# AIM-SE/AC-TSR

Hardware: AMD Instinct MI355X
Metric: user-sequences/sec fwd+bwd, AC-SASRec L=50 d=64, 1/2/4/8 MI355X (higher is better)
Workload: dtype f32; 1 GPU; ACSASRec full training step (spatial + adversarial calibrators, BASELINE configs[2]), synthetic 100000-item catalogue, B=512/GPU L=50 d=64 h=2 2 layers inner=256, CE loss, two-pass backward + Adam; global_batch=512, seq_len=50, hidden=64, heads=2, parallelism=dp1, launch=hipGraph replay per step, backward=two walks (reference protocol, trainer.py:672-686)

## Files before the change

### ac_tsr_amd/_lib.py

```python
from __future__ import annotations

import ctypes as C
import os
import subprocess

_HERE = os.path.dirname(os.path.abspath(__file__))
CSRC = os.path.join(_HERE, "csrc")
LIB_PATH = os.environ.get("ACATTN_LIB") or os.path.join(CSRC, "libacattn.so")
HEADER_PATH = os.path.join(os.path.dirname(_HERE), "include", "acattn.h")

ABI_VERSION = 32
MAX_MASKS = 8
NSTAT = 8
MASK_STRUCTURED, MASK_DENSE_LL, MASK_DENSE_L = 0, 1, 2
COMBINE = {"fixed": 0, "gate": 1, "annealing": 2}
RICH = {"none": 0, "fixed": 1, "trainable": 2}
RNG_EXPLICIT, RNG_COUNTER = 0, 1
FWD_AUTO, FWD_STREAM, FWD_STAGED, FWD_GENERAL = 0, 1, 2, 3
BWD_AUTO, BWD_STREAM, BWD_ROW = 0, 1, 2

_f = C.c_void_p


class Problem(C.Structure):
    _fields_ = [
        ("B", C.c_int32), ("L", C.c_int32), ("H", C.c_int32), ("n_heads", C.c_int32),
        ("q", _f), ("k", _f), ("v", _f), ("qa", _f), ("ka", _f), ("gate_logits", _f),
        ("mask_mode", C.c_int32), ("causal", C.c_int32), ("key_valid", _f), ("mask", _f),
        ("w_order", _f), ("b_order", _f), ("w_dist", _f), ("b_dist", _f), ("scalar", _f),
        ("adversarial", C.c_int32), ("combine_option", C.c_int32), ("anneal_rate", C.c_float),
        ("two_level", C.c_int32), ("rich_combine", C.c_int32), ("rich_ratio", _f),
        ("rng_mode", C.c_int32), ("p_drop", C.c_float), ("noise", _f), ("keep_after", _f), ("keep_before", _f),
        ("keep_mask", _f), ("seed", C.c_uint64), ("seed_device", _f), ("affine", _f), ("gate_is_prob", C.c_int32),
    ]


class FwdOut(C.Structure):
    _fields_ = [
        ("ctx_attacked", _f), ("ctx_calibrated", _f), ("attack_mask", _f), ("row_stats", _f),
        ("after_spatial", _f), ("before_spatial", _f), ("perturbed_attention", _f), ("calibrated_attention", _f),
        ("penalty_part", _f),
    ]


class BwdIO(C.Structure):
    _fields_ = [
        ("attack_mask", _f), ("row_stats", _f),
        ("d_ctx_attacked", _f), ("d_ctx_calibrated", _f), ("d_attack_mask", _f),
        ("dq", _f), ("dk", _f), ("dv", _f), ("dqa", _f), ("dka", _f), ("dgate_logits", _f),
        ("dw_order_part", _f), ("dw_dist_part", _f), ("dsmall_part", _f), ("part_stride", C.c_int32),
        ("active_qblocks", _f), ("attack_only", C.c_int32), ("workspace", _f), ("read_rows", _f),
        ("n_read_rows", C.c_int32), ("d_penalty_part", _f), ("dgate_summed", C.c_int32),
        ("d_ctx_calibrated2", _f), ("d_penalty_part2", _f), ("dqa2", _f), ("dka2", _f),
    ]


class SpatialBwdIO(C.Structure):
    _fields_ = [
        ("d_ctx", _f), ("dq", _f), ("dk", _f), ("dv", _f),
        ("dw_order_part", _f), ("dw_dist_part", _f), ("dsmall_part", _f), ("part_stride", C.c_int32),
        ("n_read_rows", C.c_int32), ("read_rows", _f), ("workspace", _f),
    ]


class CeProblem(C.Structure):
    _fields_ = [("B", C.c_int32), ("N", C.c_int32), ("H", C.c_int32), ("out", _f), ("table", _f), ("target", _f),
                ("coef_is_scalar", C.c_int32), ("coef_scale", C.c_float)]


class LnProblem(C.Structure):
    _fields_ = [("rows", C.c_int32), ("H", C.c_int32), ("residual_rows", C.c_int32), ("z", _f), ("residual", _f),
                ("gamma", _f), ("beta", _f), ("eps", C.c_float), ("p_drop", C.c_float), ("keep", _f),
                ("seed", C.c_uint64), ("seed_device", _f)]


LN_BWD_GRID = 512


class ProjProblem(C.Structure):
    _fields_ = [("rows", C.c_int32), ("H", C.c_int32), ("G", C.c_int32), ("x", _f), ("wq", _f), ("bq", _f), ("wk", _f),
                ("bk", _f), ("wv", _f), ("bv", _f), ("waq", _f), ("baq", _f), ("wak", _f), ("bak", _f), ("wg", _f),
                ("bg", _f), ("w_order", _f), ("b_order", _f), ("w_dist", _f), ("b_dist", _f), ("n_heads", C.c_int32),
                ("L", C.c_int32)]


class ProjOut(C.Structure):
    _fields_ = [("mq", _f), ("mk", _f), ("mv", _f), ("qa", _f), ("ka", _f), ("gate", _f), ("affine", _f),
                ("gate_prob", C.c_int32)]


class ProjBwdIO(C.Structure):
    _fields_ = [("dmq", _f), ("dmk", _f), ("dmv", _f), ("dqa", _f), ("dka", _f), ("dgate", _f), ("dmq_total", _f),
                ("dmk_total", _f), ("dx", _f), ("dx_init", _f), ("workspace", _f)]


ADAM_MAX_TENSORS = 64


class AdamGroup(C.Structure):
    _fields_ = [("n_tensors", C.c_int32), ("param", _f * ADAM_MAX_TENSORS), ("grad", _f * ADAM_MAX_TENSORS),
                ("exp_avg", _f * ADAM_MAX_TENSORS), ("exp_avg_sq", _f * ADAM_MAX_TENSORS), ("step", _f * ADAM_MAX_TENSORS),
                ("numel", C.c_int64 * ADAM_MAX_TENSORS)]


class TailProblem(C.Structure):
    _fields_ = [("rows", C.c_int32), ("H", C.c_int32), ("I", C.c_int32), ("ctx", _f), ("x", _f), ("wd", _f), ("bd", _f),
                ("g1", _f), ("b1", _f), ("w1", _f), ("bb1", _f), ("w2", _f), ("bb2", _f), ("g2", _f), ("b2", _f),
                ("eps1", C.c_float), ("eps2", C.c_float), ("p1", C.c_float), ("p2", C.c_float), ("keep1", _f),
                ("keep2", _f), ("seed1", C.c_uint64), ("seed2", C.c_uint64), ("seed_device", _f), ("src_index", _f),
                ("src_R", C.c_int32), ("src_L", C.c_int32), ("split_planes", _f)]


class TailSaved(C.Structure):
    _fields_ = [("h1", _f), ("st1", _f), ("a", _f), ("act", _f), ("h3", _f), ("st2", _f), ("out", _f),
                ("gelu_grad", _f)]


class TailBwdIO(C.Structure):
    _fields_ = [("d_out", _f), ("d_ctx", _f), ("d_x", _f), ("d_h1", _f), ("d_h2", _f), ("d_h3", _f), ("dgb_part", _f),
                ("workspace", _f)]


class EmbedProblem(C.Structure):
    _fields_ = [("rows", C.c_int32), ("L", C.c_int32), ("H", C.c_int32), ("n_table_rows", C.c_int64), ("idx", _f),
                ("table", _f), ("pos", _f), ("gamma", _f), ("beta", _f), ("eps", C.c_float), ("p_drop", C.c_float),
                ("keep", _f), ("seed", C.c_uint64), ("seed_device", _f), ("nonzero_out", _f), ("hot_id_plus1", C.c_int64)]


EMBED_BWD_CHUNKS = 8
PENALTY_WS_FLOATS = 1024
WGRAD_MAX_GROUP = 8
WGRAD_MAX_REDUCE = 32
SUMROWS_MAX_DEFER = 8

SYMBOLS = {
    "acattn_abi_version": (C.c_int, []),
    "acattn_calibrated_attention_bwd_gate_summed": (C.c_int, [C.POINTER(Problem), C.POINTER(BwdIO)]),
    "acattn_calibrated_attention_bwd_pair_supported": (C.c_int, [C.POINTER(Problem), C.POINTER(BwdIO)]),
    "acattn_last_error": (C.c_char_p, []),
    "acattn_fwd_algorithmic_bytes": (C.c_int64, [C.POINTER(Problem)]),
    "acattn_calibrated_attention_fwd": (C.c_int, [C.POINTER(Problem), C.POINTER(FwdOut), C.c_void_p]),
    "acattn_calibrated_attention_bwd": (C.c_int, [C.POINTER(Problem), C.POINTER(BwdIO), C.c_void_p]),
    "acattn_spatial_attention_bwd": (C.c_int, [C.POINTER(Problem), C.POINTER(SpatialBwdIO), C.c_void_p]),
    "acattn_spatial_attention_bwd_workspace_bytes": (C.c_int64, [C.POINTER(Problem)]),
    "acattn_spatial_affines": (C.c_int, [C.POINTER(Problem), _f, C.c_void_p]),
    "acattn_full_sort_ce_workspace_bytes": (C.c_int64, [C.POINTER(CeProblem)]),
    "acattn_full_sort_ce_fwd": (C.c_int, [C.POINTER(CeProblem), _f, _f, _f, C.c_void_p]),
    "acattn_full_sort_ce_fwd_dir": (C.c_int, [C.POINTER(CeProblem), _f, _f, _f, _f, C.c_void_p]),
    "acattn_full_sort_ce_bwd": (C.c_int, [C.POINTER(CeProblem), _f, _f, _f, _f, _f, C.c_void_p]),
    "acattn_full_sort_ce_products": (C.c_int, [C.c_int]),
    "acattn_linear_products": (C.c_int, [C.c_int]),
    "acattn_dropout_add_layernorm_fwd": (C.c_int, [C.POINTER(LnProblem), _f, _f, C.c_void_p]),
    "acattn_dropout_add_layernorm_bwd": (C.c_int, [C.POINTER(LnProblem), _f, _f, _f, _f, _f, C.c_void_p]),
    "acattn_embed_layernorm_fwd": (C.c_int, [C.POINTER(EmbedProblem), _f, _f, C.c_void_p]),
    "acattn_embed_layernorm_bwd": (C.c_int, [C.POINTER(EmbedProblem), _f, _f, C.c_int64, _f, _f, _f, C.c_void_p]),
    "acattn_projections_supported": (C.c_int, [C.c_int32, C.c_int32]),
    "acattn_projections_bwd_workspace_bytes": (C.c_int64, [C.POINTER(ProjProblem)]),
    "acattn_projections_fwd": (C.c_int, [C.POINTER(ProjProblem), C.POINTER(ProjOut), C.c_void_p]),
    "acattn_projections_qkv_supported": (C.c_int, [C.c_int32]),
    "acattn_projections_qkv_fwd": (C.c_int, [C.POINTER(ProjProblem), C.POINTER(ProjOut), C.c_void_p]),
    "acattn_projections_bwd": (C.c_int, [C.POINTER(ProjProblem), C.POINTER(ProjBwdIO), C.c_void_p]),
    "acattn_layer_tail_supported": (C.c_int, [C.c_int32, C.c_int32]),
    "acattn_layer_tail_fwd": (C.c_int, [C.POINTER(TailProblem), C.POINTER(TailSaved), C.c_void_p]),
    "acattn_layer_tail_bwd": (C.c_int, [C.POINTER(TailProblem), C.POINTER(TailSaved), C.POINTER(TailBwdIO), C.c_void_p]),
    "acattn_layer_tail_bwd_partial_rows": (C.c_int32, [C.c_int32]),
    "acattn_layer_tail_bwd_partial_rows_for": (C.c_int32, [C.c_int32, C.c_int32]),
    "acattn_layer_tail_bwd_workspace_bytes": (C.c_int64, [C.c_int32, C.c_int32]),
    "acattn_select_layer_tail_blocks": (C.c_int, [C.c_int]),
    "acattn_layer_tail_split_bytes": (C.c_int64, [C.c_int32, C.c_int32, C.c_int32]),
    "acattn_layer_tail_split_weights": (C.c_int, [C.POINTER(TailProblem), C.c_void_p, C.c_void_p]),
    "acattn_adam_step": (C.c_int, [C.POINTER(AdamGroup), C.c_double, C.c_double, C.c_double, C.c_double, C.c_double, _f,
                                   C.c_void_p]),
    "acattn_dense_ce_fwd": (C.c_int, [_f, C.c_int64, C.c_int64, _f, _f, _f, C.c_void_p]),
    "acattn_dense_ce_bwd": (C.c_int, [_f, _f, _f, _f, C.c_int64, C.c_int64, _f, C.c_void_p]),
    "acattn_step_inputs": (C.c_int, [C.POINTER(C.c_void_p), C.POINTER(C.c_void_p), C.POINTER(C.c_int64), C.c_int32, C.c_void_p,
                                     C.c_void_p, C.c_void_p, C.c_int32, C.c_void_p]),
    "acattn_sum_rows": (C.c_int, [_f, _f, C.c_int32, C.c_int32, C.c_int32, C.c_void_p]),
    "acattn_sum_rows_pair": (C.c_int, [_f, _f, C.c_int32, C.c_int32, C.c_int32, _f, _f, C.c_int32, C.c_int32, C.c_int32, C.c_void_p]),
    "acattn_mask_penalty_fwd": (C.c_int, [_f, C.c_int64, _f, _f, C.c_void_p]),
    "acattn_mask_penalty_partial": (C.c_int, [_f, C.c_int64, _f, C.c_void_p]),
    "acattn_mask_penalty_partial_multi": (C.c_int, [C.c_void_p, C.c_int32, C.c_int64, _f, C.c_void_p]),
    "acattn_mask_penalty_bwd_scaled_multi": (C.c_int, [C.c_void_p, _f, _f, C.c_float, C.c_int64, C.c_void_p, C.c_int32,
                                                       C.c_void_p]),
    "acattn_attacked_loss_finish": (C.c_int, [_f, C.c_int32, _f, C.c_int32, C.c_int64, C.c_float, _f, _f, C.c_int32,
                                              C.c_void_p]),
    "acattn_mask_penalty_rows": (C.c_int, [_f, C.c_int32, C.c_int32, C.c_int32, _f, C.c_void_p]),
    "acattn_attacked_loss_finish_rows": (C.c_int, [_f, C.c_int32, C.c_void_p, C.c_int32, C.c_int32, C.c_float, _f, _f, C.c_int32,
                                                  C.c_void_p]),
    "acattn_mask_penalty_drows": (C.c_int, [_f, _f, C.c_float, C.c_int32, C.c_void_p, C.c_int32, C.c_void_p]),
    "acattn_mask_penalty_drows_dir": (C.c_int, [_f, _f, C.c_float, C.c_int32, C.c_void_p, C.c_int32, _f, _f, C.c_int32, C.c_void_p]),
    "acattn_mask_penalty_bwd_scaled": (C.c_int, [_f, _f, _f, C.c_float, C.c_int64, _f, C.c_void_p]),
    "acattn_mask_penalty_bwd": (C.c_int, [_f, _f, _f, C.c_int64, _f, C.c_void_p]),
    "acattn_linear_wgrad_workspace_bytes": (C.c_int64, [C.c_int64, C.c_int32, C.c_int32]),
    "acattn_linear_wgrad_grouped": (C.c_int, [C.c_void_p, C.c_void_p, C.c_void_p, C.c_void_p, C.c_void_p, C.c_void_p,
                                               C.c_int32, C.c_int64, _f, C.c_void_p]),
    "acattn_linear_wgrad": (C.c_int, [_f, _f, C.c_int64, C.c_int32, C.c_int32, _f, _f, _f, C.c_void_p]),
    "acattn_linear_wgrad_grouped_partial": (C.c_int, [C.c_void_p, C.c_void_p, C.c_void_p, C.c_void_p, C.c_void_p, C.c_int32,
                                                       C.c_int64, C.c_void_p, C.c_void_p, C.c_void_p, C.c_void_p, C.c_void_p]),
    "acattn_linear_wgrad_reduce_many": (C.c_int, [C.c_void_p, C.c_void_p, C.c_void_p, C.c_void_p, C.c_void_p, C.c_void_p,
                                                   C.c_void_p, C.c_int32, C.c_void_p, C.c_void_p, C.c_void_p, C.c_void_p,
                                                   C.c_int32, C.c_void_p]),
    "acattn_select_forward_kernel": (C.c_int, [C.c_int]),
    "acattn_select_backward_kernel": (C.c_int, [C.c_int]),
    "acattn_calibrated_attention_bwd_workspace_bytes": (C.c_int64, [C.POINTER(Problem)]),
    "acattn_rng_materialize": (C.c_int, [C.c_int32, C.c_int32, C.c_int32, C.c_uint64, C.c_float, _f, _f, _f, _f,
                                         C.c_void_p]),
}

_lib = None


class AcattnError(RuntimeError):
    pass


def build(verbose: bool = False) -> str:
    jobs = str(min(8, os.cpu_count() or 1))
    res = subprocess.run(["make", "-C", CSRC, "-j", jobs], capture_output=not verbose, text=True)
    if res.returncode != 0:
        raise AcattnError("building libacattn.so failed:\n" + (res.stdout or "") + (res.stderr or ""))
    return LIB_PATH


def load() -> C.CDLL:
    global _lib
    if _lib is not None:
        return _lib
    if not os.path.exists(LIB_PATH):
        raise AcattnError(
            f"{LIB_PATH} is missing: the HIP extension has not been built. Run "
            "`make -C ac_tsr_amd/csrc` (or __graft_entry__.build()). There is no CPU / eager fallback.")
    lib = C.CDLL(LIB_PATH)
    for name, (res, args) in SYMBOLS.items():
        fn = getattr(lib, name)
        fn.restype = res
        fn.argtypes = args
    got = lib.acattn_abi_version()
    if got != ABI_VERSION:
        raise AcattnError(f"libacattn.so ABI {got} != binding ABI {ABI_VERSION}; rebuild")
    _lib = lib
    return lib


def check(rc: int, what: str) -> None:
    if rc == 0:
        return
    msg = load().acattn_last_error().decode()
    if rc < 0 and "not a multiple of the number of attention" in msg:
        raise ValueError(msg)
    if rc < 0 and ("unknown combine_option" in msg or "unknown rich_calibrated_combine" in msg):
        raise KeyError(msg)
    raise AcattnError(f"{what} failed (rc={rc}): {msg}")
```

### ac_tsr_amd/csrc/acattn_api.hip

```cpp
#include <stdint.h>
#include <stdio.h>
#include <string.h>

#include <algorithm>

#include "acattn_common.h"

namespace {
thread_local char g_err[256] = "";

int fail(const char* msg) {
  snprintf(g_err, sizeof(g_err), "%s", msg);
  return -1;
}

int check_problem(const acattn_problem* p) {
  if (!p) return fail("problem is NULL");
  if (p->B < 1 || p->L < 1 || p->H < 1 || p->n_heads < 1) return fail("B, L, H, n_heads must be positive");
  if (p->H % p->n_heads != 0)
    return fail("The hidden size is not a multiple of the number of attention heads");
  const int dh = p->H / p->n_heads;
  if (dh != 16 && dh != 32 && dh != 64 && dh != 128) return fail("unsupported head size: dh must be 16, 32, 64 or 128");
  if (p->L > 208) return fail("unsupported sequence length: L must be <= 208");
  if (!p->q || !p->k || !p->v) return fail("q, k, v must be non-NULL");
// ... 133 lines not shown
                                   (hipStream_t)stream);
  if (rc > 0) snprintf(g_err, sizeof(g_err), "HIP launch failed: %s", hipGetErrorString((hipError_t)rc));
  return rc;
}

static int check_ce(const acattn_ce_problem* p) {
  if (!p) return fail("ce problem is NULL");
  if (p->B < 1 || p->N < 1) return fail("B and N must be positive");
  if (p->H != 64 && p->H != 128 && p->H != 256) return fail("unsupported hidden size for the fused cross-entropy: H must be 64, 128 or 256");
  if (!p->out || !p->table || !p->target) return fail("out, table, target must be non-NULL");
  return 0;
}

int64_t acattn_full_sort_ce_workspace_bytes(const acattn_ce_problem* p) {
  if (!p || (p->H != 64 && p->H != 128 && p->H != 256)) return -1;
  return acattn_ce_ws_bytes(*p);
}

int acattn_full_sort_ce_fwd(const acattn_ce_problem* p, void* workspace, float* lse, float* row_loss, void* stream) {
  if (int rc = check_ce(p)) return rc;
  if (!workspace || !lse || !row_loss) return fail("workspace, lse, row_loss must be non-NULL");
  const int rc = acattn_launch_ce_fwd(*p, workspace, lse, row_loss, (hipStream_t)stream);
  if (rc > 0) snprintf(g_err, sizeof(g_err), "HIP launch failed: %s", hipGetErrorString((hipError_t)rc));
  return rc;
}

int acattn_full_sort_ce_fwd_dir(const acattn_ce_problem* p, void* workspace, float* lse, float* row_loss, float* dir,
                                void* stream) {
  if (int rc = check_ce(p)) return rc;
  if (!workspace || !lse || !row_loss || !dir) return fail("workspace, lse, row_loss, dir must be non-NULL");
  const int rc = acattn_launch_ce_fwd_dir(*p, workspace, lse, row_loss, dir, (hipStream_t)stream);
  if (rc > 0) snprintf(g_err, sizeof(g_err), "HIP launch failed: %s", hipGetErrorString((hipError_t)rc));
  return rc;
}

int acattn_full_sort_ce_bwd(const acattn_ce_problem* p, const float* lse, const float* coef, void* workspace,
                            float* d_out, float* d_table, void* stream) {
  if (int rc = check_ce(p)) return rc;
  if (!workspace || !lse || !coef || !d_out) return fail("workspace, lse, coef, d_out must be non-NULL");
  const int rc = acattn_launch_ce_bwd(*p, lse, coef, workspace, d_out, d_table, (hipStream_t)stream);
  if (rc > 0) snprintf(g_err, sizeof(g_err), "HIP launch failed: %s", hipGetErrorString((hipError_t)rc));
  return rc;
}

int acattn_full_sort_ce_products(int mode) { return acattn_ce_products_choice(mode); }

int acattn_linear_products(int mode) { return acattn_linear_products_choice(mode); }

static int check_ln(const acattn_ln_problem* p) {
  if (!p) return fail("ln problem is NULL");
  if (p->rows < 1) return fail("rows must be positive");
  if (p->H != 64 && p->H != 128 && p->H != 256) return fail("unsupported hidden size for the fused LayerNorm: H must be 64, 128 or 256");
  if (p->residual_rows < 1 || p->rows % p->residual_rows != 0) return fail("residual_rows must divide rows");
  if (!p->z || !p->residual || !p->gamma || !p->beta) return fail("z, residual, gamma, beta must be non-NULL");
  if (p->p_drop < 0.f || p->p_drop >= 1.f) return fail("p_drop must lie in [0, 1)");
  return 0;
}

int acattn_dropout_add_layernorm_fwd(const acattn_ln_problem* p, float* y, float* stats, void* stream) {
  if (int rc = check_ln(p)) return rc;
  if (!y || !stats) return fail("y and stats must be non-NULL");
  const int rc = acattn_launch_ln_fwd(*p, y, stats, (hipStream_t)stream);
  if (rc > 0) snprintf(g_err, sizeof(g_err), "HIP launch failed: %s", hipGetErrorString((hipError_t)rc));
  return rc;
}

int acattn_dropout_add_layernorm_bwd(const acattn_ln_problem* p, const float* dy, const float* stats, float* dz,
                                     float* dres, float* dgb_part, void* stream) {
  if (int rc = check_ln(p)) return rc;
  if (!dy || !stats) return fail("dy and stats must be non-NULL");
  const int rc = acattn_launch_ln_bwd(*p, dy, stats, dz, dres, dgb_part, (hipStream_t)stream);
  if (rc > 0) snprintf(g_err, sizeof(g_err), "HIP launch failed: %s", hipGetErrorString((hipError_t)rc));
  return rc;
}

static int check_proj(const acattn_proj_problem* p) {
  if (!p) return fail("problem must be non-NULL");
  if (p->rows < 1) return fail("rows must be positive");
  if (!acattn_proj_supported(p->H, p->G)) return fail("projections: hidden_size must be 64, 128 or 256 and the gate at most 256 wide");
  if (!p->x || !p->wq || !p->bq || !p->wk || !p->bk || !p->wv || !p->bv || !p->waq || !p->baq || !p->wak || !p->bak)
    return fail("projections: input and parameters must be non-NULL");
  if ((p->wg != nullptr) != (p->bg != nullptr) || (p->wg != nullptr) != (p->G > 0))
    return fail("projections: gate weight, bias and width go together");
  return 0;
}

int acattn_projections_supported(int32_t H, int32_t G) { return acattn_proj_supported(H, G) ? 1 : 0; }

int64_t acattn_projections_bwd_workspace_bytes(const acattn_proj_problem* p) {
  if (!p || !acattn_proj_supported(p->H, p->G)) return -1;
  return acattn_proj_bwd_ws_bytes(*p);
}

int acattn_projections_fwd(const acattn_proj_problem* p, const acattn_proj_out* out, void* stream) {
  if (int rc = check_proj(p)) return rc;
  if (!out || !out->mq || !out->mk || !out->mv || !out->qa || !out->ka) return fail("projections: outputs must be non-NULL");
  if ((p->wg != nullptr) != (out->gate != nullptr)) return fail("projections: gate output goes with the gate parameters");
  if (out->affine) {
    if (!p->w_order || !p->b_order || !p->w_dist || !p->b_dist) return fail("projections: affine planes need the spatial calibrator's parameters");
    if (p->n_heads < 1 || p->H % p->n_heads != 0 || (p->H / p->n_heads) % 16 != 0) return fail("projections: affine planes need a head size that is a multiple of 16");
    if (p->L < 1 || p->rows % p->L != 0) return fail("projections: affine planes need rows = B * L");
  }
  const int rc = acattn_launch_proj_fwd(*p, *out, (hipStream_t)stream);
  if (rc > 0) snprintf(g_err, sizeof(g_err), "HIP launch failed: %s", hipGetErrorString((hipError_t)rc));
  return rc;
}

int acattn_projections_qkv_supported(int32_t H) { return acattn_proj_qkv_supported(H) ? 1 : 0; }

int acattn_projections_qkv_fwd(const acattn_proj_problem* p, const acattn_proj_out* out, void* stream) {
  if (!p) return fail("problem must be non-NULL");
  if (p->rows < 1) return fail("rows must be positive");
  if (!acattn_proj_qkv_supported(p->H)) return fail("projections (q, k, v only): hidden_size must be 64 with the split products on");
  if (!p->x || !p->wq || !p->bq || !p->wk || !p->bk || !p->wv || !p->bv) return fail("projections: input and parameters must be non-NULL");
  if (!out || !out->mq || !out->mk || !out->mv) return fail("projections: outputs must be non-NULL");
  if (out->qa || out->ka || out->gate) return fail("projections (q, k, v only): qa, ka and gate outputs must be NULL");
  if (out->affine) {
    if (!p->w_order || !p->b_order || !p->w_dist || !p->b_dist) return fail("projections: affine planes need the spatial calibrator's parameters");
    if (p->n_heads < 1 || p->H % p->n_heads != 0 || (p->H / p->n_heads) % 16 != 0) return fail("projections: affine planes need a head size that is a multiple of 16");
    if (p->L < 1 || p->rows % p->L != 0) return fail("projections: affine planes need rows = B * L");
  }
  const int rc = acattn_launch_proj_qkv_fwd(*p, *out, (hipStream_t)stream);
  if (rc > 0) snprintf(g_err, sizeof(g_err), "HIP launch failed: %s", hipGetErrorString((hipError_t)rc));
  return rc;
}

int acattn_projections_bwd(const acattn_proj_problem* p, const acattn_proj_bwd_io* io, void* stream) {
  if (int rc = check_proj(p)) return rc;
  if (!io) return fail("io must be non-NULL");
  if (!io->dmq_total && !io->dmk_total && !io->dx) return fail("projections backward: nothing to compute");
  const int rc = acattn_launch_proj_bwd(*p, *io, (hipStream_t)stream);
  if (rc > 0) snprintf(g_err, sizeof(g_err), "HIP launch failed: %s", hipGetErrorString((hipError_t)rc));
  return rc;
}

static int check_tail(const acattn_tail_problem* p, const acattn_tail_saved* s) {
  if (!p || !s) return fail("problem and saved must be non-NULL");
  if (p->rows < 1) return fail("rows must be positive");
  if (!acattn_tail_supported(p->H, p->I)) return fail("layer tail: (hidden_size, inner_size) must be (64, 256), (64, 128), (128, 512), (128, 256) or (256, 1024)");
  if (!p->ctx || !p->x || !p->wd || !p->bd || !p->g1 || !p->b1 || !p->w1 || !p->bb1 || !p->w2 || !p->bb2 || !p->g2 || !p->b2)
    return fail("layer tail: inputs and parameters must be non-NULL");
  if (!(p->p1 >= 0.f && p->p1 < 1.f) || !(p->p2 >= 0.f && p->p2 < 1.f)) return fail("dropout probabilities must be in [0, 1)");
  if (!s->h1 || !s->st1 || !s->a || !s->h3 || !s->st2) return fail("layer tail: saved tensors must be non-NULL");
  if (p->src_index && (p->src_R < 1 || p->src_L < 1)) return fail("layer tail: src_index needs src_R, src_L >= 1");
  if (p->split_planes && p->H != 64) return fail("layer tail: split_planes is for hidden 64 only");
  if (((uintptr_t)p->split_planes & 15) != 0) return fail("layer tail: split_planes must be 16-byte aligned");
  return 0;
}

int acattn_layer_tail_supported(int32_t H, int32_t I) { return acattn_tail_supported(H, I) ? 1 : 0; }

int32_t acattn_layer_tail_bwd_partial_rows(int32_t rows) { return acattn_tail_bwd_partial_rows(rows); }
int32_t acattn_layer_tail_bwd_partial_rows_for(int32_t rows, int32_t H) { return acattn_tail_bwd_partial_rows_h(rows, H); }
int64_t acattn_layer_tail_bwd_workspace_bytes(int32_t H, int32_t I) {
  return acattn_tail_supported(H, I) ? acattn_tail_bwd_ws_bytes(H, I) : -1;
}

int64_t acattn_layer_tail_split_bytes(int32_t H, int32_t I, int32_t rows) {
  return acattn_tail_supported(H, I) && rows > 0 ? acattn_tail_split_bytes(H, I, rows) : 0;
}

int acattn_layer_tail_split_weights(const acattn_tail_problem* p, void* planes, void* stream) {
  if (!p || !planes || !p->wd || !p->w1 || !p->w2) return fail("layer tail split planes: problem, weights and planes must be non-NULL");
  if (p->H != 64 || (p->I != 256 && p->I != 128)) return fail("layer tail split planes: hidden 64, inner 256 or 128 only");
  if (((uintptr_t)planes & 15) != 0) return fail("layer tail split planes: planes must be 16-byte aligned");
  const int rc = acattn_launch_tail_split(*p, planes, (hipStream_t)stream);
  if (rc > 0) snprintf(g_err, sizeof(g_err), "HIP launch failed: %s", hipGetErrorString((hipError_t)rc));
  return rc;
}

int acattn_select_layer_tail_blocks(int nb) {
  if (nb < 0 || nb > 2) return fail("rows per wave: 0 (automatic), 1 or 2 blocks of 16");
  return acattn_select_tail_nb(nb);
}

int acattn_layer_tail_fwd(const acattn_tail_problem* p, const acattn_tail_saved* saved, void* stream) {
  if (int rc = check_tail(p, saved)) return rc;
  if (!saved->act || !saved->out) return fail("layer tail forward: act and out must be non-NULL");
  const int rc = acattn_launch_tail_fwd(*p, *saved, (hipStream_t)stream);
  if (rc > 0) snprintf(g_err, sizeof(g_err), "HIP launch failed: %s", hipGetErrorString((hipError_t)rc));
  return rc;
}

int acattn_layer_tail_bwd(const acattn_tail_problem* p, const acattn_tail_saved* saved, const acattn_tail_bwd_io* io,
                          void* stream) {
  if (int rc = check_tail(p, saved)) return rc;
  if (!io || !io->d_out) return fail("layer tail backward: d_out must be non-NULL");
  const int rc = acattn_launch_tail_bwd(*p, *saved, *io, (hipStream_t)stream);
  if (rc > 0) snprintf(g_err, sizeof(g_err), "HIP launch failed: %s", hipGetErrorString((hipError_t)rc));
  return rc;
}

int acattn_dense_ce_fwd(const float* logits, int64_t rows, int64_t N, const int64_t* target, float* lse, float* row_loss,
                        void* stream) {
  if (!logits || !target || !lse || !row_loss) return fail("dense CE: logits, target, lse, row_loss must be non-NULL");
  if (rows < 1 || N < 1) return fail("dense CE: rows and N must be positive");
  const int rc = acattn_launch_dense_ce_fwd(logits, rows, N, target, lse, row_loss, (hipStream_t)stream);
  if (rc > 0) snprintf(g_err, sizeof(g_err), "HIP launch failed: %s", hipGetErrorString((hipError_t)rc));
  return rc;
}
int acattn_dense_ce_bwd(const float* logits, const float* lse, const int64_t* target, const float* coef, int64_t rows, int64_t N,
                        float* d_logits, void* stream) {
  if (!logits || !lse || !target || !coef || !d_logits) return fail("dense CE backward: every pointer must be non-NULL");
  if (rows < 1 || N < 1) return fail("dense CE: rows and N must be positive");
  const int rc = acattn_launch_dense_ce_bwd(logits, lse, target, coef, rows, N, d_logits, (hipStream_t)stream);
  if (rc > 0) snprintf(g_err, sizeof(g_err), "HIP launch failed: %s", hipGetErrorString((hipError_t)rc));
  return rc;
}

int acattn_step_inputs(const void* const* src, void* const* dst, const int64_t* bytes, int32_t n_copies, int64_t* counter,
                       const int64_t* item_length, int64_t* last_row, int32_t n_rows, void* stream) {
  if (n_copies < 0 || n_copies > ACATTN_MAX_COPIES) return fail("step inputs: 0 .. ACATTN_MAX_COPIES copies");
  if (n_copies > 0 && (!src || !dst || !bytes)) return fail("step inputs: src, dst, bytes must be non-NULL");
  for (int k = 0; k < n_copies; ++k)
    if (bytes[k] > 0 && (!src[k] || !dst[k])) return fail("step inputs: NULL copy operand");
  if ((item_length == nullptr) != (last_row == nullptr)) return fail("step inputs: item_length and last_row come together");
  if (last_row && n_rows < 1) return fail("step inputs: n_rows must be positive");
  const int rc = acattn_launch_step_inputs(src, dst, bytes, n_copies, counter, item_length, last_row, n_rows, (hipStream_t)stream);
  if (rc > 0) snprintf(g_err, sizeof(g_err), "HIP launch failed: %s", hipGetErrorString((hipError_t)rc));
  return rc;
}

int acattn_sum_rows(const float* x, float* out, int32_t batch, int32_t R, int32_t C, void* stream) {
  if (!x || !out) return fail("x and out must be non-NULL");
  if (batch < 1 || R < 1 || C < 1) return fail("batch, R, C must be positive");
  const int rc = acattn_launch_sum_rows(x, out, batch, R, C, (hipStream_t)stream);
  if (rc > 0) snprintf(g_err, sizeof(g_err), "HIP launch failed: %s", hipGetErrorString((hipError_t)rc));
  return rc;
}

int acattn_sum_rows_pair(const float* x1, float* out1, int32_t batch1, int32_t R1, int32_t C1, const float* x2, float* out2,
                         int32_t batch2, int32_t R2, int32_t C2, void* stream) {
  if (!x1 || !out1 || !x2 || !out2) return fail("x and out must be non-NULL");
  if (batch1 < 1 || R1 < 1 || C1 < 1 || batch2 < 1 || R2 < 1 || C2 < 1) return fail("batch, R, C must be positive");
  const int rc = acattn_launch_sum_rows_pair(x1, out1, batch1, R1, C1, x2, out2, batch2, R2, C2, (hipStream_t)stream);
  if (rc > 0) snprintf(g_err, sizeof(g_err), "HIP launch failed: %s", hipGetErrorString((hipError_t)rc));
  return rc;
}

static int check_embed(const acattn_embed_problem* p) {
  if (!p) return fail("embed problem is NULL");
  if (p->rows < 1 || p->L < 1 || p->rows % p->L != 0) return fail("rows must be a positive multiple of L");
  if (p->H != 64 && p->H != 128 && p->H != 256) return fail("unsupported hidden size for the fused embedding front end: H must be 64, 128 or 256");
  if (p->n_table_rows < 1) return fail("n_table_rows must be positive");
  if (!p->idx || !p->table || !p->gamma || !p->beta) return fail("idx, table, gamma, beta must be non-NULL");
  if (p->p_drop < 0.f || p->p_drop >= 1.f) return fail("p_drop must lie in [0, 1)");
  return 0;
}

// ... 229 lines not shown
```

### ac_tsr_amd/csrc/acattn_common.h

```cpp
#pragma once
#include <hip/hip_runtime.h>
#include <stdint.h>

#include <type_traits>

#include "acattn.h"

typedef float f4 __attribute__((ext_vector_type(4)));
typedef float f4u __attribute__((ext_vector_type(4), aligned(4)));

#define ACATTN_NEG_INF (-__builtin_inff())
#define ACATTN_MASK_FILL (-10000.0f)
#define ACATTN_LOG_EPS (1e-24f)

__device__ __forceinline__ float quad_sum(float x) {
  auto r = __builtin_amdgcn_permlane16_swap(__float_as_uint(x), __float_as_uint(x), false, false);
  x = __uint_as_float(r[0]) + __uint_as_float(r[1]);
  auto s = __builtin_amdgcn_permlane32_swap(__float_as_uint(x), __float_as_uint(x), false, false);
  return __uint_as_float(s[0]) + __uint_as_float(s[1]);
}

__device__ __forceinline__ float quad_max(float x) {
  auto r = __builtin_amdgcn_permlane16_swap(__float_as_uint(x), __float_as_uint(x), false, false);
  x = fmaxf(__uint_as_float(r[0]), __uint_as_float(r[1]));
// ... 177 lines not shown
  x ^= x >> 16;
  x += key.b;
  return (rng_word(x, 0xB5297A4Du, 0x85EBCA77u) >> 12) & 0xFu;
}

__device__ __forceinline__ f4 keep_scale4(uint32_t bits, float keep_scale) {
  f4 s;
#pragma unroll
  for (int r = 0; r < 4; ++r) s[r] = ((bits >> r) & 1u) ? keep_scale : 0.f;
  return s;
}
__device__ __forceinline__ int sbit(uint32_t bits, int idx) {
  int m = __builtin_amdgcn_sbfe(bits, idx, 1);
  asm("" : "+v"(m));
  return m;
}
__device__ __forceinline__ float keep_and(float x, uint32_t bits, int r) {
  return __uint_as_float(__float_as_uint(x) & (uint32_t)sbit(bits, r));
}

__device__ __forceinline__ void store_out4(float* p, const f4 v) { __builtin_nontemporal_store(v, (f4*)p); }
__device__ __forceinline__ void store_out1(float* p, const float v) { __builtin_nontemporal_store(v, p); }

__device__ __forceinline__ bool qblock_has_ctx(const acattn_bwd_io& IO, int b, int qb) {
  if (IO.active_qblocks) return (IO.active_qblocks[b] >> qb) & 1u;
  if (IO.read_rows) {
    for (int r = 0; r < IO.n_read_rows; ++r)
      if ((int)(IO.read_rows[(size_t)b * IO.n_read_rows + r] >> 4) == qb) return true;
    return false;
  }
  return true;
}

__device__ __forceinline__ bool qblock_active(const acattn_bwd_io& IO, int b, int qb) {
  if (IO.d_attack_mask || IO.d_penalty_part) return true;
  if (IO.active_qblocks) return (IO.active_qblocks[b] >> qb) & 1u;
  if (IO.read_rows) {
    for (int r = 0; r < IO.n_read_rows; ++r)
      if ((int)(IO.read_rows[(size_t)b * IO.n_read_rows + r] >> 4) == qb) return true;
    return false;
  }
  return true;
}

__device__ __forceinline__ void decode_block(int bid, int B, int nh, int& b, int& h) {
  if ((B & 7) == 0) {
    const int grp = bid / (8 * nh), rem = bid - grp * 8 * nh;
    h = rem >> 3;
    b = grp * 8 + (rem & 7);
  } else {
    b = bid / nh;
    h = bid - b * nh;
  }
}

int acattn_launch_fwd(const acattn_problem& p, const acattn_fwd_out& o, hipStream_t stream);
int acattn_fwd_kernel_choice(int which);
int acattn_bwd_kernel_choice(int which);
int64_t acattn_bwd_stream_ws_bytes(const acattn_problem& p);
int acattn_launch_bwd(const acattn_problem& p, const acattn_bwd_io& io, hipStream_t stream);
bool acattn_bwd_gate_summed(const acattn_problem& p, const acattn_bwd_io& io);
bool acattn_bwd_pair_supported(const acattn_problem& p, const acattn_bwd_io& io);
int64_t acattn_spatial_bwd_ws_bytes(const acattn_problem& p);
int acattn_launch_spatial_bwd(const acattn_problem& p, const acattn_spatial_bwd_io& io, hipStream_t stream);
int acattn_launch_spatial_affines(const acattn_problem& p, float* affine, hipStream_t stream);
int acattn_launch_rng(int B, int nh, int L, uint64_t seed, float p_drop, float* noise, uint8_t* keep_after,
                      uint8_t* keep_mask, uint8_t* keep_before, hipStream_t stream);
int64_t acattn_ce_ws_bytes(const acattn_ce_problem& p);
int acattn_launch_ce_fwd(const acattn_ce_problem& p, void* ws, float* lse, float* row_loss, hipStream_t stream);
int acattn_launch_ce_fwd_dir(const acattn_ce_problem& p, void* ws, float* lse, float* row_loss, float* dir,
                             hipStream_t stream);
int acattn_launch_ce_bwd(const acattn_ce_problem& p, const float* lse, const float* coef, void* ws, float* d_out,
                         float* d_table, hipStream_t stream);
int acattn_launch_ln_fwd(const acattn_ln_problem& p, float* y, float* stats, hipStream_t stream);
int acattn_launch_ln_bwd(const acattn_ln_problem& p, const float* dy, const float* stats, float* dz, float* dres,
                         float* dgb_part, hipStream_t stream);
int acattn_launch_sum_rows(const float* x, float* out, int batch, int R, int C, hipStream_t stream);
int acattn_launch_sum_rows_pair(const float* x1, float* out1, int batch1, int R1, int C1, const float* x2, float* out2,
                                int batch2, int R2, int C2, hipStream_t stream);
void acattn_set_error(const char* msg);
bool acattn_proj_supported(int H, int G);
int64_t acattn_proj_bwd_ws_bytes(const acattn_proj_problem& p);
int acattn_launch_proj_fwd(const acattn_proj_problem& p, const acattn_proj_out& o, hipStream_t stream);
bool acattn_proj_qkv_supported(int H);
int acattn_launch_proj_qkv_fwd(const acattn_proj_problem& p, const acattn_proj_out& o, hipStream_t stream);
int acattn_launch_proj_bwd(const acattn_proj_problem& p, const acattn_proj_bwd_io& io, hipStream_t stream);
bool acattn_tail_supported(int H, int I);
int acattn_tail_bwd_partial_rows(int rows);
int acattn_tail_bwd_partial_rows_h(int rows, int H);
int64_t acattn_tail_bwd_ws_bytes(int H, int I);
int acattn_select_tail_nb(int nb);
int64_t acattn_tail_split_bytes(int H, int I, int rows);
int acattn_launch_tail_split(const acattn_tail_problem& p, void* planes, hipStream_t stream);
int acattn_launch_tail_fwd(const acattn_tail_problem& p, const acattn_tail_saved& s, hipStream_t stream);
int acattn_launch_tail_bwd(const acattn_tail_problem& p, const acattn_tail_saved& s, const acattn_tail_bwd_io& io,
                           hipStream_t stream);
int64_t acattn_linear_wgrad_ws_bytes(int64_t M, int K, int N);
int acattn_launch_linear_wgrad(const float* const* x, const float* const* dy, const int* K, const int* N,
                               float* const* dw, float* const* db, int n_items, int64_t M, void* ws, hipStream_t stream,
                               int* P_out = nullptr, long long* w_off_out = nullptr, long long* b_off_out = nullptr);
int acattn_launch_linear_wgrad_reduce_many(const float* const* part_w, const float* const* part_b, const int* K, const int* N,
                                           const int* P, float* const* dw, float* const* db, int n_items,
                                           const float* const* sr_x, float* const* sr_out, const int* sr_R, const int* sr_C,
                                           int n_sr, hipStream_t stream);
int acattn_launch_embed_fwd(const acattn_embed_problem& p, float* y, float* stats, hipStream_t stream);
int acattn_launch_embed_bwd(const acattn_embed_problem& p, const float* dy, const float* stats, int64_t padding_idx,
                            float* d_table, float* d_pos_part, float* dgb_part, hipStream_t stream);
int acattn_launch_penalty_fwd(const float* m, int64_t n, float* ws, float* norm, hipStream_t stream);
int acattn_launch_penalty_partial(const float* m, int64_t n, float* part, hipStream_t stream);
void acattn_penalty_written_set(bool v);
bool acattn_penalty_written();
int acattn_launch_penalty_rows(const float* m, int B, int nh, int L, float* pen, hipStream_t stream);
int acattn_launch_attacked_loss_finish_rows(const float* row_loss, int B, const float* const* pen, int n_masks, int count,
                                            float weight, float* out, float* scale_buf, int n_scale, hipStream_t stream);
int acattn_launch_penalty_drows(const float* norms, const float* d_loss, float scale, int count, float* const* d_pen,
                                int n_masks, hipStream_t stream, const float* dir = nullptr, float* d_out = nullptr, int n_dir = 0);
int acattn_launch_attacked_loss_finish(const float* row_loss, int B, const float* part, int n_masks, int64_t mask_numel,
                                       float weight, float* out, float* scale_buf, int n_scale, hipStream_t stream);
int acattn_launch_penalty_bwd_scaled(const float* m, const float* norm, const float* d_loss, float scale, int64_t n,
                                     float* d_m, hipStream_t stream);
int acattn_launch_penalty_bwd(const float* m, const float* norm, const float* d_norm, int64_t n, float* d_m,
                              hipStream_t stream);
int acattn_launch_zero(float* p, size_t n, hipStream_t stream);
int64_t acattn_ce6_rows_bytes(const acattn_ce_problem& p);
int acattn_launch_ce6_sweep(const acattn_ce_problem& p, const float* lse, const float* coef, float* slab, float* d_table,
                            float2* part, void* rows_ws, int n_wg, int n_left, bool dir, hipStream_t stream);
int acattn_launch_ce6_onehot_reduce(const acattn_ce_problem& p, const float* coef, const float* slab, int n_slabs, float* d_out,
                                    float* d_table, hipStream_t stream);
int acattn_launch_ce6_fwd_sweep(const acattn_ce_problem& p, float2* part, void* rows_ws, int n_wg, int n_left, hipStream_t stream);
int acattn_ce_products_choice(int mode);
int acattn_linear_products_choice(int mode);
int acattn_launch_dense_ce_fwd(const float* logits, int64_t rows, int64_t N, const int64_t* target, float* lse, float* row_loss,
                               hipStream_t stream);
int acattn_launch_dense_ce_bwd(const float* logits, const float* lse, const int64_t* target, const float* coef, int64_t rows,
                               int64_t N, float* d_logits, hipStream_t stream);
int acattn_launch_step_inputs(const void* const* src, void* const* dst, const int64_t* bytes, int n, int64_t* counter,
                              const int64_t* item_length, int64_t* last_row, int n_rows, hipStream_t stream);
int acattn_launch_penalty_partial_multi(const float* const* m, int n_masks, int64_t n, float* part, hipStream_t stream);
int acattn_launch_penalty_bwd_scaled_multi(const float* const* m, const float* norms, const float* d_loss, float scale,
                                           int64_t n, float* const* d_m, int n_masks, hipStream_t stream);
int acattn_launch_adam_step(const acattn_adam_group& g, double lr, double beta1, double beta2, double eps,
                            double weight_decay, int* done, hipStream_t stream);
```

### ac_tsr_amd/csrc/acattn_proj.hip

```cpp
#include <stdlib.h>
#include <string.h>

#include <algorithm>
#include <type_traits>

#include "acattn_common.h"
#include "acattn_split.h"
#include "acattn_wstage.h"

namespace {

template <int NB>
struct Rows {
  int row[NB];
  bool ok[NB];
};

template <int NB>
__device__ __forceinline__ Rows<NB> wave_rows(int R) {
  Rows<NB> w;
  const int c = threadIdx.x & 15;
#pragma unroll
  for (int nb = 0; nb < NB; ++nb) {
    const int r = (blockIdx.x * NB + nb) * 16 + c;
// ... 751 lines not shown
  f4 in[NB][DT], tot[NB][DT];
  auto zero = [&](f4 (&v)[NB][DT]) {
#pragma unroll
    for (int nb = 0; nb < NB; ++nb)
#pragma unroll
      for (int t = 0; t < DT; ++t) v[nb][t] = f4{0.f, 0.f, 0.f, 0.f};
  };
  auto masked_store_rows = [&](float* out, const f4 (&v)[NB][DT]) {
#pragma unroll
    for (int nb = 0; nb < NB; ++nb)
      if (W.ok[nb])
#pragma unroll
        for (int t = 0; t < DT; ++t) *(f4*)(out + (size_t)W.row[nb] * H + 16 * t + 4 * g) = v[nb][t];
  };
  if (h_dmq) load_rows<DT, NB>(IO.dmq, W, g, tot); else zero(tot);
  if (h_dqa) load_rows<DT, NB>(IO.dqa, W, g, in);
  st.commit();
  if (h_dqa) staged_keep<DT, NB, false>(st, waqT, nullptr, in, tot, after_qa);
  if (h_gate) {
    static_assert(DT == KT || DT == 2 * KT, "");
    for (int kt = 0; kt < GT; ++kt) {
      f4 d[NB];
#pragma unroll
      for (int nb = 0; nb < NB; ++nb) {
        const int j0 = 16 * kt + 4 * g;
        const float* src = IO.dgate + (size_t)W.row[nb] * P.G + j0;
        f4 v = {0.f, 0.f, 0.f, 0.f};
        if (j0 + 3 < P.G) {
          v = *(const f4u*)src;
        } else {
#pragma unroll
          for (int r = 0; r < 4; ++r)
            if (j0 + r < P.G) v[r] = src[r];
        }
        d[nb] = v;
      }
#pragma unroll
      for (int half = 0; half < DT / KT; ++half) {
        f4 frag[KT], b;
        st.fetch(frag, b);
        if (half + 1 < DT / KT)
          st.request_cols(wgT + (size_t)(16 * KT) * ldg * (half + 1), ldg, kt);
        else if (kt + 1 < GT)
          st.request_cols(wgT, ldg, kt + 1);
        else
          after_q_total();
        PIN_ORDER();
#pragma unroll
        for (int r = 0; r < 4; ++r)
#pragma unroll
          for (int nt = 0; nt < KT; ++nt)
#pragma unroll
            for (int nb = 0; nb < NB; ++nb) {
              if (half == 0) tot[nb][nt] = mfma16(frag[nt][r], d[nb][r], tot[nb][nt]);
              else tot[nb][DT - KT + nt] = mfma16(frag[nt][r], d[nb][r], tot[nb][DT - KT + nt]);
            }
        PIN_ORDER();
        st.commit();
      }
    }
  }
  if (h_qt) masked_store_rows(IO.dmq_total, tot);
  if (h_dmk) load_rows<DT, NB>(IO.dmk, W, g, tot); else zero(tot);
  if (h_dka) {
    load_rows<DT, NB>(IO.dka, W, g, in);
    staged_keep<DT, NB, false>(st, wakT, nullptr, in, tot, after_k_total);
  }
  if (h_kt) masked_store_rows(IO.dmk_total, tot);
  if (h_dx) {
    f4 (&dx)[NB][DT] = in;
    if (IO.dx_init) load_rows<DT, NB>(IO.dx_init, W, g, dx); else zero(dx);
    staged_keep<DT, NB, false>(st, wkT, nullptr, tot, dx, [&] { first(wqT); });
    load_rows<DT, NB>(IO.dmq_total, W, g, tot);
    staged_keep<DT, NB, false>(st, wqT, nullptr, tot, dx, [&] { if (h_dmv) first(wvT); else st.has_bias = false; });
    if (h_dmv) {
      load_rows<DT, NB>(IO.dmv, W, g, tot);
      staged_keep<DT, NB, false>(st, wvT, nullptr, tot, dx, [&] { st.has_bias = false; });
    }
    masked_store_rows(IO.dx, dx);
  }
}

constexpr int SPW = 4;
constexpr int SPLIT_MAT = 4 * 2 * 3 * 64;
constexpr int SPLIT_LDS = 6 * SPLIT_MAT * (int)sizeof(b8);

__device__ __forceinline__ int kperm(int s, int g, int j) { return 32 * s + 16 * (j >> 2) + 4 * g + (j & 3); }

template <bool T>
__device__ __forceinline__ void split_raw(const float* w, int n_out, int nt, int c, int g, float (&v)[2][8]) {
#pragma unroll
  for (int s = 0; s < 2; ++s) {
    if constexpr (!T) {
      const float* row = w + (size_t)min(16 * nt + c, n_out - 1) * 64 + 32 * s + 4 * g;
      const f4 lo = *(const f4*)row, hi = *(const f4*)(row + 16);
#pragma unroll
      for (int r = 0; r < 4; ++r) {
        v[s][r] = lo[r];
        v[s][4 + r] = hi[r];
      }
    } else {
#pragma unroll
      for (int j = 0; j < 8; ++j) {
        const int k = kperm(s, g, j);
        const float t = w[(size_t)min(k, n_out - 1) * 64 + 16 * nt + c];
        v[s][j] = k < n_out ? t : 0.f;
      }
    }
  }
}

__device__ __forceinline__ void split_store(const float (&v)[2][8], b8* mat, int nt, int lane) {
#pragma unroll
  for (int s = 0; s < 2; ++s) {
    b8 p[3];
    split8(v[s], p[0], p[1], p[2]);
#pragma unroll
    for (int q = 0; q < 3; ++q) mat[((nt * 2 + s) * 3 + q) * 64 + lane] = p[q];
  }
}

template <int NB>
__device__ __forceinline__ void split_rows(const f4 (&v)[NB][4], b8 (&b)[NB][2][3]) {
#pragma unroll
  for (int nb = 0; nb < NB; ++nb)
#pragma unroll
    for (int s = 0; s < 2; ++s) {
      float x[8];
#pragma unroll
      for (int r = 0; r < 4; ++r) {
        x[r] = v[nb][2 * s][r];
        x[4 + r] = v[nb][2 * s + 1][r];
      }
      split8(x, b[nb][s][0], b[nb][s][1], b[nb][s][2]);
    }
}

template <int NB, int NT = 4>
__device__ __forceinline__ void split_product(const b8* mat, int lane, const b8 (&b)[NB][2][3], f4 (&acc)[NB][4]) {
#pragma unroll
  for (int nt = 0; nt < NT; ++nt) {
    b8 a[2][3];
#pragma unroll
    for (int s = 0; s < 2; ++s)
#pragma unroll
      for (int q = 0; q < 3; ++q) a[s][q] = mat[((nt * 2 + s) * 3 + q) * 64 + lane];
#pragma unroll
    for (int s = 0; s < 2; ++s)
#pragma unroll
      for (int nb = 0; nb < NB; ++nb) acc[nb][nt] = mfma_split(a[s], b[nb][s], acc[nb][nt]);
  }
}

template <int NB>
__device__ __forceinline__ Rows<NB> split_rows_of(int R, int wave) {
  Rows<NB> w;
  const int c = threadIdx.x & 15;
#pragma unroll
  for (int nb = 0; nb < NB; ++nb) {
    const int r = ((blockIdx.x * SPW + wave) * NB + nb) * 16 + c;
    w.ok[nb] = r < R;
    w.row[nb] = r < R ? r : R - 1;
  }
  return w;
}

template <int NB>
__global__ void __launch_bounds__(64 * SPW) proj_split_fwd_kernel(const acattn_proj_problem P, const acattn_proj_out O) {
// ... 107 lines not shown
  split_product<NB>(wsp + 2 * SPLIT_MAT, lane, xs, acc);
  store_rows<4, NB>(O.mv, W, g, acc);
}

template <int NB, int MODE>
__global__ void __launch_bounds__(64 * SPW) proj_split_bwd_kernel(const acattn_proj_problem P, const acattn_proj_bwd_io IO) {
  extern __shared__ b8 wsp[];
  const bool h_dmq = MODE == 1 || (MODE == 0 && IO.dmq), h_dmk = MODE == 1 || (MODE == 0 && IO.dmk);
  const bool h_dmv = MODE == 1 || (MODE == 0 && IO.dmv);
  const bool h_dqa = MODE != 0 || IO.dqa, h_dka = MODE != 0 || IO.dka, h_dx = MODE != 0 || IO.dx;
  const bool h_qt = MODE != 0 || IO.dmq_total, h_kt = MODE != 0 || IO.dmk_total;
  const bool gate = MODE != 2 && IO.dgate && P.wg;
  const int lane = threadIdx.x & 63, wave = threadIdx.x >> 6, c = lane & 15, g = lane >> 4;
  const Rows<NB> W = split_rows_of<NB>(P.rows, wave);
  {
    const float* src[6] = {P.waq, gate ? P.wg : P.waq, P.wq, P.wak, P.wk, P.wv};
    const bool need[6] = {h_dqa, gate, h_dx, h_dka, h_dx, h_dx && h_dmv};
    float v[6][2][8];
#pragma unroll
    for (int m = 0; m < 6; ++m)
      if (need[m]) split_raw<true>(src[m], m == 1 ? P.G : 64, wave, c, g, v[m]);
#pragma unroll
    for (int m = 0; m < 6; ++m)
      if (need[m]) split_store(v[m], wsp + m * SPLIT_MAT, wave, lane);
  }
  auto zero = [&](f4 (&v)[NB][4]) {
#pragma unroll
    for (int nb = 0; nb < NB; ++nb)
#pragma unroll
      for (int t = 0; t < 4; ++t) v[nb][t] = f4{0.f, 0.f, 0.f, 0.f};
  };
  f4 in[NB][4], dq[NB][4], dk[NB][4], dx[NB][4];
  b8 bs[NB][2][3];
  if (IO.dx_init && h_dx) load_rows<4, NB>(IO.dx_init, W, g, dx); else zero(dx);
  if (h_dmq) load_rows<4, NB>(IO.dmq, W, g, dq); else zero(dq);
  if (h_dqa) load_rows<4, NB>(IO.dqa, W, g, in);
  __syncthreads();

  if (h_dqa) {
    split_rows<NB>(in, bs);
    split_product<NB>(wsp, lane, bs, dq);
  }
  if (gate) {
#pragma unroll
    for (int nb = 0; nb < NB; ++nb)
#pragma unroll
      for (int s = 0; s < 2; ++s) {
        float x[8];
#pragma unroll
        for (int j = 0; j < 8; ++j) {
          const int k = kperm(s, g, j);
          const float t = IO.dgate[(size_t)W.row[nb] * P.G + min(k, P.G - 1)];
          x[j] = k < P.G ? t : 0.f;
        }
        split8(x, bs[nb][s][0], bs[nb][s][1], bs[nb][s][2]);
      }
    split_product<NB>(wsp + SPLIT_MAT, lane, bs, dq);
  }
  if (h_qt) store_rows<4, NB>(IO.dmq_total, W, g, dq);
  if (h_dx) {
    split_rows<NB>(dq, bs);
    split_product<NB>(wsp + 2 * SPLIT_MAT, lane, bs, dx);
  }

  if (h_dmk) load_rows<4, NB>(IO.dmk, W, g, dk); else zero(dk);
  if (h_dka) {
    load_rows<4, NB>(IO.dka, W, g, in);
    split_rows<NB>(in, bs);
    split_product<NB>(wsp + 3 * SPLIT_MAT, lane, bs, dk);
  }
  if (h_kt) store_rows<4, NB>(IO.dmk_total, W, g, dk);
  if (h_dx) {
    split_rows<NB>(dk, bs);
    split_product<NB>(wsp + 4 * SPLIT_MAT, lane, bs, dx);
    if (h_dmv) {
      load_rows<4, NB>(IO.dmv, W, g, in);
      split_rows<NB>(in, bs);
      split_product<NB>(wsp + 5 * SPLIT_MAT, lane, bs, dx);
    }
    store_rows<4, NB>(IO.dx, W, g, dx);
  }
}

int rows_per_wave(int rows) {
  static const int forced = getenv("ACATTN_PROJ_ROWS_PER_WAVE") ? atoi(getenv("ACATTN_PROJ_ROWS_PER_WAVE")) : 0;
  if (forced == 16 || forced == 32) return forced;
  return rows >= 16384 ? 32 : 16;
}

}

bool acattn_proj_supported(int H, int G) { return (H == 64 || H == 128 || H == 256) && G >= 0 && G <= 256; }

int64_t acattn_proj_bwd_ws_bytes(const acattn_proj_problem& p) {
  if (p.H == 64) return 0;
  return ((int64_t)5 * p.H * p.H + (int64_t)p.H * ((p.G + 15) & ~15)) * (int64_t)sizeof(float);
}

namespace {
template <int H>
int launch_wide_fwd(const acattn_proj_problem& p, const acattn_proj_out& o, hipStream_t stream) {
#ifdef ACATTN_PROJ_NB1
  constexpr int NB = 1;
#else
  constexpr int NB = H == 128 ? 2 : 1;
#endif
  static const bool per_wave = getenv("ACATTN_PROJ_PER_WAVE") != nullptr;
  if (!per_wave) {
    const int blocks = (p.rows + 16 * NB * NWV - 1) / (16 * NB * NWV);
    hipLaunchKernelGGL((proj_staged_fwd_kernel<H, NB>), dim3(blocks), dim3(64 * NWV), 0, stream, p, o);
    return (int)hipGetLastError();
  }
  const int blocks = (p.rows + 16 * NB - 1) / (16 * NB);
  hipLaunchKernelGGL((proj_wide_fwd_kernel<H, NB>), dim3(blocks), dim3(64), 0, stream, p, o);
  return (int)hipGetLastError();
}
template <int H>
int launch_wide_bwd(const acattn_proj_problem& p, const acattn_proj_bwd_io& io, hipStream_t stream) {
  constexpr int NB = H == 128 ? 2 : 1;
  if (!io.workspace) {
    acattn_set_error("projections backward at hidden 128 / 256 needs acattn_proj_bwd_io.workspace");
    return -1;
  }
  if (io.dx && !io.dmq_total) {
    acattn_set_error("projections backward at hidden 128 / 256: dx needs dmq_total (it is read back as a source of dx)");
    return -1;
  }
  float* wt = (float*)io.workspace;
  TransposeJob J;
  const float* src[6] = {p.wq, p.wk, p.wv, p.waq, p.wak, p.wg};
  for (int k = 0; k < 6; ++k) {
    J.src[k] = src[k];
    J.n_out[k] = k < 5 ? p.H : p.G;
  }
  const int max_out = std::max(p.H, (p.G + 15) & ~15);
  hipLaunchKernelGGL(transpose_weights_kernel, dim3(max_out / 16, p.H / 16, p.wg ? 6 : 5), dim3(256), 0, stream, J, p.H, wt);
  const bool outs = io.dx && io.dmq_total && io.dmk_total, attack = io.dqa && io.dka;
  const bool all_in = attack && io.dmq && io.dmk && io.dmv && (io.dgate || !p.wg);
  const bool attack_only = attack && !io.dmq && !io.dmk && !io.dmv && !io.dgate;
  const int mode = !outs ? 0 : all_in ? 1 : attack_only ? 2 : 0;
  static const bool per_wave = getenv("ACATTN_PROJ_PER_WAVE") != nullptr;
  if (!per_wave) {
    const int wgs = (p.rows + 16 * NB * NWV - 1) / (16 * NB * NWV);
    if (mode == 1)
      hipLaunchKernelGGL((proj_staged_bwd_kernel<H, NB, 1>), dim3(wgs), dim3(64 * NWV), 0, stream, p, io, (const float*)wt);
    else if (mode == 2)
      hipLaunchKernelGGL((proj_staged_bwd_kernel<H, NB, 2>), dim3(wgs), dim3(64 * NWV), 0, stream, p, io, (const float*)wt);
    else
      hipLaunchKernelGGL((proj_staged_bwd_kernel<H, NB, 0>), dim3(wgs), dim3(64 * NWV), 0, stream, p, io, (const float*)wt);
    return (int)hipGetLastError();
  }
  const int blocks = (p.rows + 16 * NB - 1) / (16 * NB);
  if (mode == 1)
    hipLaunchKernelGGL((proj_wide_bwd_kernel<H, NB, 1>), dim3(blocks), dim3(64), 0, stream, p, io, (const float*)wt);
  else if (mode == 2)
    hipLaunchKernelGGL((proj_wide_bwd_kernel<H, NB, 2>), dim3(blocks), dim3(64), 0, stream, p, io, (const float*)wt);
  else
    hipLaunchKernelGGL((proj_wide_bwd_kernel<H, NB, 0>), dim3(blocks), dim3(64), 0, stream, p, io, (const float*)wt);
  return (int)hipGetLastError();
}
}

namespace {
int g_linear_products = -1;
int linear_products() {
  if (g_linear_products < 0) {
    const char* e = getenv("ACATTN_LINEAR_PRODUCTS");
    g_linear_products = e && !strcmp(e, "fp32") ? 0 : 1;
  }
  return g_linear_products;
}
bool use_split(const acattn_proj_problem& p) { return p.H == 64 && (!p.wg || p.G <= 64) && linear_products() == 1; }

template <class K>
bool allow_split_lds(K kern) {
  return hipFuncSetAttribute((const void*)kern, hipFuncAttributeMaxDynamicSharedMemorySize, SPLIT_LDS) == hipSuccess;
}

template <int NB>
int launch_split_fwd(const acattn_proj_problem& p, const acattn_proj_out& o, hipStream_t stream) {
  static const bool lds_ok = allow_split_lds(proj_split_fwd_kernel<NB>);
  if (!lds_ok) return (int)hipErrorInvalidValue;
  const int wgs = (p.rows + 16 * NB * SPW - 1) / (16 * NB * SPW);
  hipLaunchKernelGGL((proj_split_fwd_kernel<NB>), dim3(wgs), dim3(64 * SPW), SPLIT_LDS, stream, p, o);
  return (int)hipGetLastError();
}

template <int NB, int MODE>
int launch_split_bwd(const acattn_proj_problem& p, const acattn_proj_bwd_io& io, hipStream_t stream) {
  static const bool lds_ok = allow_split_lds(proj_split_bwd_kernel<NB, MODE>);
  if (!lds_ok) return (int)hipErrorInvalidValue;
  const int wgs = (p.rows + 16 * NB * SPW - 1) / (16 * NB * SPW);
  hipLaunchKernelGGL((proj_split_bwd_kernel<NB, MODE>), dim3(wgs), dim3(64 * SPW), SPLIT_LDS, stream, p, io);
  return (int)hipGetLastError();
}
}

int acattn_linear_products_choice(int mode) {
  const int old = linear_products();
  if (mode >= 0 && mode <= 1) g_linear_products = mode;
  return old;
}

int acattn_launch_proj_fwd(const acattn_proj_problem& p, const acattn_proj_out& o, hipStream_t stream) {
  if (p.H == 128) return launch_wide_fwd<128>(p, o, stream);
  if (p.H == 256) return launch_wide_fwd<256>(p, o, stream);
  const int rpw = rows_per_wave(p.rows), blocks = (p.rows + rpw - 1) / rpw;
  if (use_split(p)) return rpw == 32 ? launch_split_fwd<2>(p, o, stream) : launch_split_fwd<1>(p, o, stream);
  if (rpw == 32)
    hipLaunchKernelGGL((proj_fwd_kernel<64, 2>), dim3(blocks), dim3(64), 0, stream, p, o);
  else
    hipLaunchKernelGGL((proj_fwd_kernel<64, 1>), dim3(blocks), dim3(64), 0, stream, p, o);
  return (int)hipGetLastError();
}

bool acattn_proj_qkv_supported(int H) { return H == 64 && linear_products() == 1; }

namespace {
template <int NB>
int launch_split_qkv_fwd(const acattn_proj_problem& p, const acattn_proj_out& o, hipStream_t stream) {
  static const bool lds_ok = hipFuncSetAttribute((const void*)proj_split_qkv_fwd_kernel<NB>,
                                                 hipFuncAttributeMaxDynamicSharedMemorySize, SPLIT_QKV_LDS) == hipSuccess;
  if (!lds_ok) return (int)hipErrorInvalidValue;
  const int wgs = (p.rows + 16 * NB * SPW - 1) / (16 * NB * SPW);
  hipLaunchKernelGGL((proj_split_qkv_fwd_kernel<NB>), dim3(wgs), dim3(64 * SPW), SPLIT_QKV_LDS, stream, p, o);
  return (int)hipGetLastError();
}
}

int acattn_launch_proj_qkv_fwd(const acattn_proj_problem& p, const acattn_proj_out& o, hipStream_t stream) {
  if (!acattn_proj_qkv_supported(p.H)) {
    acattn_set_error("projections (q, k, v only): hidden_size must be 64 with the split products on");
    return -1;
  }
  return rows_per_wave(p.rows) == 32 ? launch_split_qkv_fwd<2>(p, o, stream) : launch_split_qkv_fwd<1>(p, o, stream);
}

int acattn_launch_proj_bwd(const acattn_proj_problem& p, const acattn_proj_bwd_io& io, hipStream_t stream) {
  if (p.H == 128) return launch_wide_bwd<128>(p, io, stream);
  if (p.H == 256) return launch_wide_bwd<256>(p, io, stream);
  const int rpw = rows_per_wave(p.rows), blocks = (p.rows + rpw - 1) / rpw;
  const bool outs = io.dx && io.dmq_total && io.dmk_total, attack = io.dqa && io.dka;
  const bool all_in = attack && io.dmq && io.dmk && io.dmv && (io.dgate || !p.wg);
  const bool attack_only = attack && !io.dmq && !io.dmk && !io.dmv && !io.dgate;
  const int mode = !outs ? 0 : all_in ? 1 : attack_only ? 2 : 0;
  if (use_split(p)) {
    if (rpw == 32) {
      if (mode == 1) return launch_split_bwd<2, 1>(p, io, stream);
      if (mode == 2) return launch_split_bwd<2, 2>(p, io, stream);
      return launch_split_bwd<2, 0>(p, io, stream);
    }
    if (mode == 1) return launch_split_bwd<1, 1>(p, io, stream);
    if (mode == 2) return launch_split_bwd<1, 2>(p, io, stream);
    return launch_split_bwd<1, 0>(p, io, stream);
  }
#define LAUNCH(NB, MODE) hipLaunchKernelGGL((proj_bwd_kernel<64, NB, MODE>), dim3(blocks), dim3(64), 0, stream, p, io)
  if (rpw == 32) {
    if (mode == 1) LAUNCH(2, 1); else if (mode == 2) LAUNCH(2, 2); else LAUNCH(2, 0);
  } else {
    if (mode == 1) LAUNCH(1, 1); else if (mode == 2) LAUNCH(1, 2); else LAUNCH(1, 0);
  }
#undef LAUNCH
  return (int)hipGetLastError();
}
```

### ac_tsr_amd/csrc/acattn_split.h

```cpp
#pragma once

#include "acattn_common.h"

namespace {

typedef __bf16 b8 __attribute__((ext_vector_type(8)));

#define ACATTN_SPLIT_TERMS(X) X(0, 2) X(1, 1) X(2, 0) X(0, 1) X(1, 0) X(0, 0)

__device__ __forceinline__ f4 mfma_bf(const b8 a, const b8 b, const f4 c) {
  return __builtin_amdgcn_mfma_f32_16x16x32_bf16(a, b, c, 0, 0, 0);
}

__device__ __forceinline__ void split8(const float (&x)[8], b8& p0, b8& p1, b8& p2) {
#pragma unroll
  for (int j = 0; j < 8; ++j) {
    const __bf16 a = (__bf16)x[j];
    const float r1 = x[j] - (float)a;
    const __bf16 b = (__bf16)r1;
    const float r2 = r1 - (float)b;
    p0[j] = a;
    p1[j] = b;
    p2[j] = (__bf16)r2;
  }
}

__device__ __forceinline__ f4 mfma_split(const b8 (&a)[3], const b8 (&b)[3], f4 acc) {
#define ACATTN_SPLIT_TERM(p, q) acc = mfma_bf(a[p], b[q], acc);
  ACATTN_SPLIT_TERMS(ACATTN_SPLIT_TERM)
#undef ACATTN_SPLIT_TERM
  return acc;
}

}
```

### ac_tsr_amd/csrc/acattn_tail.hip

```cpp
#include <stdlib.h>
#include <string.h>

#include <algorithm>

#include "acattn_common.h"
#include "acattn_rowops.h"
#include "acattn_split.h"
#include "acattn_wstage.h"

int acattn_tail_bwd_partial_rows(int rows);
int acattn_tail_bwd_partial_rows_h(int rows, int H);

namespace {

int g_tail_nb = getenv("ACATTN_TAIL_BLOCKS") ? atoi(getenv("ACATTN_TAIL_BLOCKS")) : 0;
bool split_slabs(int rows) {
  static const int limit = getenv("ACATTN_TAIL_SPLIT_ROWS") ? atoi(getenv("ACATTN_TAIL_SPLIT_ROWS")) : 4096;
  return g_tail_nb == 0 && rows <= limit;
}
#ifndef ACATTN_TAIL64_WAVES
#define ACATTN_TAIL64_WAVES 3
#endif
bool staged64(int rows) {
  static const bool per_wave = getenv("ACATTN_TAIL_PER_WAVE") != nullptr;
// ... 412 lines not shown
        const size_t o = (size_t)W.row[nb] * H + 16 * t + 4 * g;
        z[t] = *(const f4*)(S.h1 + o);
        res[t] = *(const f4*)(P.x + (size_t)W.src[nb] * H + 16 * t + 4 * g);
        keep[t] = row_keep_scale(P.p1, P.keep1, P.seed1 + step, W.row[nb], 4 * t + g, H);
      }
      const float2 st = *(const float2*)(S.st1 + 2 * (size_t)W.row[nb]);
      ln_backward<DT>(z, res, keep, P.g1, st.x, st.y, da[nb], W.ok[nb], g, dz, acc_g, acc_b);
#pragma unroll
      for (int t = 0; t < DT; ++t) {
        const size_t o = (size_t)W.row[nb] * H + 16 * t + 4 * g;
        dh1[nb][t] = dz[t] * keep[t];
        if (W.ok[nb]) {
          if (IO.d_x) store_grad(IO.d_x + (size_t)W.src[nb] * H + 16 * t + 4 * g, dz[t], P.src_index != nullptr);
          if (IO.d_h1) *(f4*)(IO.d_h1 + o) = dh1[nb][t];
        }
      }
    }
    if (part) {
      store_partial<DT>(part, acc_g, c, g);
      store_partial<DT>(part + H, acc_b, c, g);
    }
  }
  if (IO.d_ctx) {
    f4 dc[NB][DT];
#pragma unroll
    for (int nb = 0; nb < NB; ++nb)
#pragma unroll
      for (int nt = 0; nt < DT; ++nt) dc[nb][nt] = f4{0.f, 0.f, 0.f, 0.f};
    f4 wdt[DT][DT];
#pragma unroll
    for (int nt = 0; nt < DT; ++nt)
#pragma unroll
      for (int t = 0; t < DT; ++t)
#pragma unroll
        for (int r = 0; r < 4; ++r) wdt[nt][t][r] = P.wd[(size_t)(16 * t + 4 * g + r) * H + 16 * nt + c];
#pragma unroll
    for (int t = 0; t < DT; ++t)
#pragma unroll
      for (int r = 0; r < 4; ++r)
#pragma unroll
        for (int nt = 0; nt < DT; ++nt)
#pragma unroll
          for (int nb = 0; nb < NB; ++nb) dc[nb][nt] = mfma16(wdt[nt][t][r], dh1[nb][t][r], dc[nb][nt]);
#pragma unroll
    for (int nb = 0; nb < NB; ++nb)
      if (W.ok[nb])
#pragma unroll
        for (int nt = 0; nt < DT; ++nt) store_grad(IO.d_ctx + (size_t)W.src[nb] * H + 16 * nt + 4 * g, dc[nb][nt], P.src_index != nullptr);
  }
}


template <int I>
struct TailPlanes {
  static constexpr int SQ = 64 * 64 * 3 / 8, RECT = I * 64 * 3 / 8;
  static constexpr int FWD_D = 0, FWD_1 = SQ, FWD_2 = SQ + RECT;
  static constexpr int BWD_D = SQ + 2 * RECT, BWD_1 = 2 * SQ + 2 * RECT, BWD_2 = 2 * SQ + 3 * RECT;
  static constexpr int TOTAL = 2 * SQ + 4 * RECT;
};

__device__ __forceinline__ int tail_kperm(int s, int g, int j) { return 32 * s + 16 * (j >> 2) + 4 * g + (j & 3); }

template <int I>
__global__ void __launch_bounds__(256) tail_split_planes_kernel(const float* wd, const float* w1, const float* w2, b8* planes) {
  using L = TailPlanes<I>;
  const int mtx = blockIdx.y, which = mtx % 3;
  const bool T = mtx >= 3;
  const float* w = which == 0 ? wd : which == 1 ? w1 : w2;
  const int M = which == 0 ? 64 : ((which == 1) != T ? I : 64), K = (which == 0 ? 64 * 64 : 64 * I) / M, KS = K / 32;
  b8* dst = planes + (mtx == 0 ? L::FWD_D : mtx == 1 ? L::FWD_1 : mtx == 2 ? L::FWD_2 : mtx == 3 ? L::BWD_D : mtx == 4 ? L::BWD_1 : L::BWD_2);
  const int idx = blockIdx.x * 256 + threadIdx.x;
  if (idx >= (M / 16) * KS * 64) return;
  const int lane = idx & 63, f = idx >> 6, mt = f / KS, s = f % KS, c = lane & 15, g = lane >> 4, m = 16 * mt + c;
  float x[8];
#pragma unroll
  for (int j = 0; j < 8; ++j) {
    const int k = tail_kperm(s, g, j);
    x[j] = T ? w[(size_t)k * M + m] : w[(size_t)m * K + k];
  }
  b8 p[3];
  split8(x, p[0], p[1], p[2]);
#pragma unroll
  for (int q = 0; q < 3; ++q) dst[((size_t)f * 3 + q) * 64 + lane] = p[q];
}

template <int KS>
__device__ __forceinline__ void load_frag(const b8* mat, int mt, int s, int lane, b8 (&a)[3]) {
#pragma unroll
  for (int q = 0; q < 3; ++q) a[q] = mat[((mt * KS + s) * 3 + q) * 64 + lane];
}

__device__ __forceinline__ void split_tiles(const f4 lo, const f4 hi, b8 (&b)[3]) {
  float x[8];
#pragma unroll
  for (int r = 0; r < 4; ++r) {
    x[r] = lo[r];
    x[4 + r] = hi[r];
  }
  split8(x, b[0], b[1], b[2]);
}

template <int NB>
__device__ __forceinline__ void split_rows64(const f4 (&v)[NB][4], b8 (&b)[NB][2][3]) {
#pragma unroll
  for (int nb = 0; nb < NB; ++nb)
#pragma unroll
    for (int s = 0; s < 2; ++s) split_tiles(v[nb][2 * s], v[nb][2 * s + 1], b[nb][s]);
}

template <int NB>
__device__ __forceinline__ void split_square(const b8* mat, int lane, const b8 (&b)[NB][2][3], f4 (&acc)[NB][4]) {
#pragma unroll
  for (int nt = 0; nt < 4; ++nt)
#pragma unroll
    for (int s = 0; s < 2; ++s) {
      b8 w[3];
      load_frag<2>(mat, nt, s, lane, w);
#pragma unroll
      for (int nb = 0; nb < NB; ++nb) acc[nb][nt] = mfma_split(w, b[nb][s], acc[nb][nt]);
    }
}

template <int H, int I, int NB, int NW = 1>
__global__ void __launch_bounds__(64 * NW) tail_split_fwd_kernel(const acattn_tail_problem P, const acattn_tail_saved S) {
  static_assert(H == 64 && (NW == 1 || NB == 1), "hidden 64; the slab split works on one row block");
  using L = TailPlanes<I>;
  constexpr int DT = 4, NP = I / 32, NJ = NP / NW;
  static_assert(NP % NW == 0 && NJ >= 1, "whole pairs per wave");
  const int lane = threadIdx.x & 63, c = lane & 15, g = lane >> 4;
  const int wave = NW > 1 ? __builtin_amdgcn_readfirstlane(threadIdx.x >> 6) : 0;
  const Rows<NB> W = wave_rows<NB>(P);
  const uint64_t step = P.seed_device ? *P.seed_device : 0ull;
  const b8* planes = (const b8*)P.split_planes;
  const b8 *pw1 = planes + L::FWD_1, *pw2 = planes + L::FWD_2;

  struct W1Pair {
    b8 w[2][2][3];
    f4 b[2];
  };
  auto load_w1 = [&](int p, W1Pair& d) {
#pragma unroll
    for (int tt = 0; tt < 2; ++tt) {
#pragma unroll
      for (int s = 0; s < 2; ++s) load_frag<2>(pw1, 2 * p + tt, s, lane, d.w[tt][s]);
      d.b[tt] = *(const f4*)(P.bb1 + 32 * p + 16 * tt + 4 * g);
    }
  };
  W1Pair w1b[2];
  load_w1(wave, w1b[0]);

  f4 h1[NB][DT], a[NB][DT];
  {
    f4 cb[NB][DT], res[NB][DT], bd[DT], g1[DT], b1[DT];
#pragma unroll
    for (int nb = 0; nb < NB; ++nb)
#pragma unroll
      for (int t = 0; t < DT; ++t) {
        cb[nb][t] = *(const f4*)(P.ctx + (size_t)W.src[nb] * H + 16 * t + 4 * g);
        res[nb][t] = *(const f4*)(P.x + (size_t)W.src[nb] * H + 16 * t + 4 * g);
      }
    load_cols<DT>(P.bd, g, bd);
    load_cols<DT>(P.g1, g, g1);
    load_cols<DT>(P.b1, g, b1);
    b8 cs[NB][2][3];
    split_rows64<NB>(cb, cs);
#pragma unroll
// ... 1258 lines not shown
  }
  const int nb = rows_per_wave(p.rows) / 16;
  const int blocks = (p.rows + 16 * nb - 1) / (16 * nb);
  if (p.split_planes) {
    if (nb == 1 && split_slabs(p.rows))
      hipLaunchKernelGGL((tail_split_fwd_kernel<H, I, 1, 4>), dim3(blocks), dim3(256), 0, stream, p, s);
    else if (nb == 2)
      hipLaunchKernelGGL((tail_split_fwd_kernel<H, I, 2>), dim3(blocks), dim3(64), 0, stream, p, s);
    else
      hipLaunchKernelGGL((tail_split_fwd_kernel<H, I, 1>), dim3(blocks), dim3(64), 0, stream, p, s);
    return (int)hipGetLastError();
  }
  if (nb == 1 && split_slabs(p.rows)) {
    hipLaunchKernelGGL((tail_fwd_kernel<H, I, 1, 4>), dim3(blocks), dim3(256), 0, stream, p, s);
    return (int)hipGetLastError();
  }
  if (nb == 2)
    hipLaunchKernelGGL((tail_fwd_kernel<H, I, 2>), dim3(blocks), dim3(64), 0, stream, p, s);
  else
    hipLaunchKernelGGL((tail_fwd_kernel<H, I, 1>), dim3(blocks), dim3(64), 0, stream, p, s);
  return (int)hipGetLastError();
}

template <int H, int I>
int launch_bwd(const acattn_tail_problem& p, const acattn_tail_saved& s, const acattn_tail_bwd_io& io, hipStream_t stream) {
  if (staged64(p.rows)) {
    if (!io.workspace) {
      acattn_set_error("layer tail backward: this row count needs acattn_tail_bwd_io.workspace (acattn_layer_tail_bwd_workspace_bytes)");
      return -1;
    }
    float* ws = (float*)io.workspace;
    hipLaunchKernelGGL(tail_transpose_kernel, dim3(I / 16, I / 16, 3), dim3(256), 0, stream, p.w1, p.w2, p.wd, H, I, ws);
    const int wgs = (p.rows + 16 * NWV - 1) / (16 * NWV);
    if (s.gelu_grad)
      hipLaunchKernelGGL((tail_chunked_bwd_kernel<H, I, true>), dim3(wgs), dim3(64 * NWV), 0, stream, p, s, io, (const float*)ws);
    else
      hipLaunchKernelGGL((tail_chunked_bwd_kernel<H, I, false>), dim3(wgs), dim3(64 * NWV), 0, stream, p, s, io, (const float*)ws);
    return (int)hipGetLastError();
  }
  const int nb = rows_per_wave(p.rows) / 16;
  const int blocks = acattn_tail_bwd_partial_rows(p.rows);
  if (p.split_planes && !(nb == 1 && split_slabs(p.rows))) {
    if (nb == 2)
      hipLaunchKernelGGL((tail_split_bwd_kernel<H, I, 2>), dim3(blocks), dim3(64), 0, stream, p, s, io);
    else
      hipLaunchKernelGGL((tail_split_bwd_kernel<H, I, 1>), dim3(blocks), dim3(64), 0, stream, p, s, io);
    return (int)hipGetLastError();
  }
  if (nb == 1 && split_slabs(p.rows)) {
    hipLaunchKernelGGL((tail_bwd_kernel<H, I, 1, 4>), dim3(blocks), dim3(256), 0, stream, p, s, io);
    return (int)hipGetLastError();
  }
  if (nb == 2)
    hipLaunchKernelGGL((tail_bwd_kernel<H, I, 2>), dim3(blocks), dim3(64), 0, stream, p, s, io);
  else
    hipLaunchKernelGGL((tail_bwd_kernel<H, I, 1>), dim3(blocks), dim3(64), 0, stream, p, s, io);
  return (int)hipGetLastError();
}

}

bool acattn_tail_supported(int H, int I) {
  return (H == 64 && (I == 256 || I == 128)) || (H == 128 && (I == 512 || I == 256)) || (H == 256 && I == 1024);
}

int acattn_tail_bwd_partial_rows(int rows) { return (rows + rows_per_wave(rows) - 1) / rows_per_wave(rows); }
int acattn_tail_bwd_partial_rows_h(int rows, int H) {
  return (H > 64 || staged64(rows)) ? (rows + 15) / 16 : acattn_tail_bwd_partial_rows(rows);
}
int64_t acattn_tail_bwd_ws_bytes(int H, int I) { return ((int64_t)2 * H * I + (int64_t)H * H) * (int64_t)sizeof(float); }

int64_t acattn_tail_split_bytes(int H, int I, int rows) {
  if (!tail_split_products(H, I, rows)) return 0;
  return (int64_t)(I == 256 ? TailPlanes<256>::TOTAL : TailPlanes<128>::TOTAL) * (int64_t)sizeof(b8);
}

int acattn_launch_tail_split(const acattn_tail_problem& p, void* planes, hipStream_t stream) {
  if (p.H == 64 && p.I == 256) return launch_split_planes<256>(p, planes, stream);
  if (p.H == 64 && p.I == 128) return launch_split_planes<128>(p, planes, stream);
  acattn_set_error("layer tail split planes: hidden 64, inner 256 or 128 only");
  return -1;
}

int acattn_select_tail_nb(int nb) {
  const int prev = g_tail_nb;
  g_tail_nb = nb;
  return prev;
}

int acattn_launch_tail_fwd(const acattn_tail_problem& p, const acattn_tail_saved& s, hipStream_t stream) {
  if (p.H == 64 && p.I == 256) return launch_fwd<64, 256>(p, s, stream);
  if (p.H == 64 && p.I == 128) return launch_fwd<64, 128>(p, s, stream);
  if (p.H == 128 && p.I == 512) return launch_wide_fwd<128, 512>(p, s, stream);
  if (p.H == 128 && p.I == 256) return launch_wide_fwd<128, 256>(p, s, stream);
  if (p.H == 256 && p.I == 1024) return launch_wide_fwd<256, 1024>(p, s, stream);
  acattn_set_error("layer tail: unsupported (hidden_size, inner_size)");
  return -1;
}

int acattn_launch_tail_bwd(const acattn_tail_problem& p, const acattn_tail_saved& s, const acattn_tail_bwd_io& io,
                           hipStream_t stream) {
  if (p.H == 64 && p.I == 256) return launch_bwd<64, 256>(p, s, io, stream);
  if (p.H == 64 && p.I == 128) return launch_bwd<64, 128>(p, s, io, stream);
  if (p.H == 128 && p.I == 512) return launch_wide_bwd<128, 512>(p, s, io, stream);
  if (p.H == 128 && p.I == 256) return launch_wide_bwd<128, 256>(p, s, io, stream);
  if (p.H == 256 && p.I == 1024) return launch_wide_bwd<256, 1024>(p, s, io, stream);
  acattn_set_error("layer tail: unsupported (hidden_size, inner_size)");
  return -1;
}
```

### ac_tsr_amd/layers.py

```python
from __future__ import annotations

import copy
import math
from typing import List, Optional

import torch
import torch.nn as nn
import torch.nn.functional as F

from . import fused_ln, ops
from . import tail
from .linear import projections, projections_qkv, skinny_linear
from .ops import AttentionConfig, ExplicitRandomness, StructuredMask
from .state import state_of


class AttackRMultiHeadAttention(nn.Module):

    def __init__(self, n_heads, hidden_size, hidden_dropout_prob, attn_dropout_prob, layer_norm_eps, use_order,
                 use_distance):
        super().__init__()
        if hidden_size % n_heads != 0:
            raise ValueError(
                "The hidden size (%d) is not a multiple of the number of attention "
                "heads (%d)" % (hidden_size, n_heads))
        self.num_attention_heads = n_heads
        self.attention_head_size = int(hidden_size / n_heads)
        self.all_head_size = self.num_attention_heads * self.attention_head_size
        self.sqrt_attention_head_size = math.sqrt(self.attention_head_size)

        self.query = nn.Linear(hidden_size, self.all_head_size)
        self.key = nn.Linear(hidden_size, self.all_head_size)
        self.value = nn.Linear(hidden_size, self.all_head_size)

        self.use_order = use_order
        self.use_distance = use_distance
        if self.use_order:
            self.order_affine = nn.Linear(2 * self.attention_head_size, 1)
        if self.use_distance:
            self.distance_affine = nn.Linear(2 * self.attention_head_size, 1)
            self.scalar = nn.Parameter(torch.randn(1))

        self.attack_query_transform = nn.Linear(self.all_head_size, self.all_head_size)
        self.attack_key_transform = nn.Linear(self.all_head_size, self.all_head_size)

        self.attn_dropout_prob = attn_dropout_prob
        self.dense = nn.Linear(hidden_size, hidden_size)
        self.LayerNorm = nn.LayerNorm(hidden_size, eps=layer_norm_eps)
        self.out_dropout = nn.Dropout(hidden_dropout_prob)

    def project(self, input_tensor):
        mq = skinny_linear(input_tensor, self.query)
        mk = skinny_linear(input_tensor, self.key)
        mv = skinny_linear(input_tensor, self.value)
        qa = skinny_linear(mq, self.attack_query_transform)
        ka = skinny_linear(mk, self.attack_key_transform)
        return mq, mk, mv, qa, ka

    def calibrator_params(self):
        p = {}
        if self.use_order:
            p.update(w_order=self.order_affine.weight, b_order=self.order_affine.bias)
        if self.use_distance:
            p.update(w_dist=self.distance_affine.weight, b_dist=self.distance_affine.bias, scalar=self.scalar)
        return p

    def output(self, context_layer, input_tensor, _keep=None):
        hidden_states = skinny_linear(context_layer, self.dense)
        if hidden_states.is_cuda and fused_ln.supported(hidden_states.shape[-1]):
            return fused_ln.dropout_add_layer_norm(hidden_states, input_tensor, self.LayerNorm, self.out_dropout.p,
                                                   self.training, _keep)
        if _keep is not None:
            hidden_states = hidden_states * (_keep.to(hidden_states.dtype) / (1.0 - self.out_dropout.p))
        else:
            hidden_states = self.out_dropout(hidden_states)
        return self.LayerNorm(hidden_states + input_tensor)


class FeedForward(nn.Module):

    def __init__(self, hidden_size, inner_size, hidden_dropout_prob, hidden_act, layer_norm_eps):
        super().__init__()
        self.dense_1 = nn.Linear(hidden_size, inner_size)
        self.intermediate_act_fn = self.get_hidden_act(hidden_act)
        self.dense_2 = nn.Linear(inner_size, hidden_size)
        self.LayerNorm = nn.LayerNorm(hidden_size, eps=layer_norm_eps)
        self.dropout = nn.Dropout(hidden_dropout_prob)

    def get_hidden_act(self, act):
        ACT2FN = {
            "gelu": self.gelu,
            "relu": F.relu,
            "swish": self.swish,
            "tanh": torch.tanh,
            "sigmoid": torch.sigmoid,
        }
        return ACT2FN[act]

    def gelu(self, x):
        return F.gelu(x)

    def swish(self, x):
        return x * torch.sigmoid(x)

    def forward(self, input_tensor, _keep=None):
        hidden_states = skinny_linear(self.intermediate_act_fn(skinny_linear(input_tensor, self.dense_1)), self.dense_2)
        if hidden_states.is_cuda and fused_ln.supported(hidden_states.shape[-1]):
            return fused_ln.dropout_add_layer_norm(hidden_states, input_tensor, self.LayerNorm, self.dropout.p,
                                                   self.training, _keep)
        if _keep is not None:
            hidden_states = hidden_states * (_keep.to(hidden_states.dtype) / (1.0 - self.dropout.p))
        else:
            hidden_states = self.dropout(hidden_states)
        return self.LayerNorm(hidden_states + input_tensor)


class AttackRTransformerLayer(nn.Module):

    def __init__(self, n_heads, hidden_size, intermediate_size, hidden_dropout_prob, attn_dropout_prob, hidden_act,
                 layer_norm_eps, combine_option='fixed', use_order=True, use_distance=True, two_level=True,
                 rich_calibrated_combine='fixed', seq_length=50, adversarial=True):
        super().__init__()
        self.adversarial = bool(adversarial)
        self.hidden_size = hidden_size
        self.attack_attention = AttackRMultiHeadAttention(
            n_heads, hidden_size, hidden_dropout_prob, attn_dropout_prob, layer_norm_eps,
            use_order=use_order, use_distance=use_distance)
        self.two_level = two_level
        self.rich_calibrated_combine = rich_calibrated_combine
        if self.rich_calibrated_combine == 'trainable':
            self.rich_calibrated_combine_ratio = torch.nn.Parameter(torch.FloatTensor([0.5]), requires_grad=True)
        self.combine_option = combine_option
        if self.combine_option == 'gate':
            self.gate = torch.nn.Linear(hidden_size, seq_length)
        self.combine_ratio = 0.5
        self.feed_forward = FeedForward(hidden_size, intermediate_size, hidden_dropout_prob, hidden_act, layer_norm_eps)
        self.anneal_step = 0

    def _config(self) -> AttentionConfig:
        rate = 1.0
        if self.combine_option == 'annealing':
            rate = math.exp(-self.anneal_step / 100000)
            self.anneal_step += 1
        return AttentionConfig(n_heads=self.attack_attention.num_attention_heads, combine_option=self.combine_option,
                               two_level=self.two_level, rich_calibrated_combine=self.rich_calibrated_combine,
                               adversarial=self.adversarial, anneal_rate=rate)

    def forward(self, hidden_states, attention_mask, return_attention_prob=False, return_all_attention_prob=False,
                _rnd=None, _need_attacked=True, _attack_upstream=True, _rows=None):
        att = self.attack_attention
        cal = att.calibrator_params()
        if not self.adversarial:
            return self._forward_spatial_only(hidden_states, attention_mask, return_attention_prob, return_all_attention_prob,
                                              _rnd, _rows)
        mq, mk, mv, qa, ka, gate_logits, hidden_res, extras = projections(
            hidden_states, att.query, att.key, att.value, att.attack_query_transform, att.attack_key_transform,
            self.gate if self.combine_option == 'gate' else None, attack_upstream=_attack_upstream,
            spatial=(cal.get("w_order"), cal.get("b_order"), cal.get("w_dist"), cal.get("b_dist"), att.num_attention_heads))
        cfg = self._config()
        core_rnd = None
        if _rnd is not None:
            core_rnd = ExplicitRandomness(noise=_rnd.noise, keep_after=getattr(_rnd, "keep_after", None),
                                          keep_mask=getattr(_rnd, "keep_mask", None),
                                          keep_before=getattr(_rnd, "keep_before", None))
        p_drop = att.attn_dropout_prob if (self.training or (core_rnd is not None and core_rnd.keep_after is not None)) else 0.0
        want_probs = return_all_attention_prob or return_attention_prob
        ctx_att, ctx_cal, attack_mask, probs = ops.calibrated_attention(
            mq, mk, mv, qa, ka, gate_logits, attention_mask, cfg, p_drop=p_drop, rnd=core_rnd, want_probs=want_probs,
            seed_tensor=state_of(self).seed_tensor if core_rnd is None else None, read_rows=_rows,
            attack_upstream=_attack_upstream, state=state_of(self), rich_ratio=getattr(self, "rich_calibrated_combine_ratio", None),
            **extras, **cal)
        residual = hidden_res
        if _rows is not None:
            index = _rows.unsqueeze(-1).expand(-1, -1, hidden_states.shape[-1])
            pick = lambda t: None if t is None else t.gather(1, index)
            picks_itself = ctx_cal.is_cuda and tail.supported(att, self.feed_forward) and tail.fused_supported(att, self.feed_forward)
            if not picks_itself:
                residual = pick(hidden_res)
        else:
            pick = lambda t: t

        def branch(ctx_layer, keep_out, keep_ffn):
            one_launch = ctx_layer.is_cuda and tail.supported(att, self.feed_forward) and tail.fused_supported(att, self.feed_forward)
            fused = one_launch or (ctx_layer.is_cuda and torch.is_grad_enabled() and tail.supported(att, self.feed_forward))
            if one_launch and _rows is not None:
                return tail.layer_tail(ctx_layer, hidden_res, att, self.feed_forward, pick(keep_out), pick(keep_ffn),
                                       pick=_rows)
            ctx_layer, keep_out, keep_ffn = pick(ctx_layer), pick(keep_out), pick(keep_ffn)
            if fused:
                return tail.layer_tail(ctx_layer, residual, att, self.feed_forward, keep_out, keep_ffn)
            return self.feed_forward(att.output(ctx_layer, residual, keep_out), keep_ffn)

        attacked_feedforward_output = None
        if _need_attacked:
            attacked_feedforward_output = branch(ctx_att, getattr(_rnd, "keep_out_att", None),
                                                 getattr(_rnd, "keep_ffn_att", None))
        calibrated_feedforward_output = branch(ctx_cal, getattr(_rnd, "keep_out_cal", None),
                                               getattr(_rnd, "keep_ffn_cal", None))
        combined_attention_prob = probs.get("calibrated_attention")
        if return_all_attention_prob:
            all_attention_prob = {
                'before_spatial': probs["before_spatial"],
                'after_spatial': probs["after_spatial"],
                'perturbed_mask': attack_mask,
                'perturbed_attention': probs["perturbed_attention"],
                'calibrated_attention': probs["calibrated_attention"],
            }
            return (attacked_feedforward_output, calibrated_feedforward_output, attack_mask, combined_attention_prob,
                    all_attention_prob)
        return attacked_feedforward_output, calibrated_feedforward_output, attack_mask, combined_attention_prob

    def _forward_spatial_only(self, hidden_states, attention_mask, return_attention_prob, return_all_attention_prob, _rnd, _rows):
        if return_attention_prob or return_all_attention_prob:
            raise ValueError("adversarial=False: the spatial-only attention core has no probability dumps "
                             "(return_attention_prob / return_all_attention_prob need the adversarial calibrator)")
        att = self.attack_attention
        cal = att.calibrator_params()
        mq, mk, mv, hidden_res, extras = projections_qkv(
            hidden_states, att.query, att.key, att.value,
            spatial=(cal.get("w_order"), cal.get("b_order"), cal.get("w_dist"), cal.get("b_dist"), att.num_attention_heads))
        cfg = self._config()
        core_rnd = None
        if _rnd is not None:
            core_rnd = ExplicitRandomness(keep_after=getattr(_rnd, "keep_after", None))
        p_drop = att.attn_dropout_prob if (self.training or (core_rnd is not None and core_rnd.keep_after is not None)) else 0.0
        _, ctx_cal, _, _ = ops.calibrated_attention(
            mq, mk, mv, None, None, None, attention_mask, cfg, p_drop=p_drop, rnd=core_rnd,
            seed_tensor=state_of(self).seed_tensor if core_rnd is None else None, read_rows=_rows, attack_upstream=False,
            state=state_of(self), **extras, **cal)
        keep_out, keep_ffn = getattr(_rnd, "keep_out_cal", None), getattr(_rnd, "keep_ffn_cal", None)
        can_tail = ctx_cal.is_cuda and tail.supported(att, self.feed_forward)
        one_launch = can_tail and tail.fused_supported(att, self.feed_forward)
        if _rows is not None:
            index = _rows.unsqueeze(-1).expand(-1, -1, hidden_states.shape[-1])
            pick = lambda t: None if t is None else t.gather(1, index)
            if one_launch:
                out = tail.layer_tail(ctx_cal, hidden_res, att, self.feed_forward, pick(keep_out), pick(keep_ffn), pick=_rows)
                return None, out, None, None
            ctx_cal, hidden_res, keep_out, keep_ffn = pick(ctx_cal), pick(hidden_res), pick(keep_out), pick(keep_ffn)
        if one_launch or (can_tail and torch.is_grad_enabled()):
            out = tail.layer_tail(ctx_cal, hidden_res, att, self.feed_forward, keep_out, keep_ffn)
        else:
            out = self.feed_forward(att.output(ctx_cal, hidden_res, keep_out), keep_ffn)
        return None, out, None, None


class AttackRTransformerEncoder(nn.Module):

    def __init__(self, n_layers=2, n_heads=2, hidden_size=64, inner_size=256, hidden_dropout_prob=0.5,
                 attn_dropout_prob=0.5, hidden_act='gelu', layer_norm_eps=1e-12, combine_option='fixed', use_order=True,
                 use_distance=True, two_level=True, rich_calibrated_combine='fixed', seq_length=50, adversarial=True):
        super().__init__()
        self.adversarial = bool(adversarial)
        layer = AttackRTransformerLayer(
            n_heads, hidden_size, inner_size, hidden_dropout_prob, attn_dropout_prob, hidden_act, layer_norm_eps,
            combine_option, use_order=use_order, use_distance=use_distance, two_level=two_level,
            rich_calibrated_combine=rich_calibrated_combine, seq_length=seq_length, adversarial=adversarial)
        self.layer = nn.ModuleList([copy.deepcopy(layer) for _ in range(n_layers)])

    def forward(self, hidden_states, attention_mask, output_all_encoded_layers=True, return_attention_prob=False,
                return_all_attention_prob=False, _rnds: Optional[List] = None, _last_rows=None):
        if _last_rows is not None and output_all_encoded_layers:
            raise ValueError("_last_rows needs output_all_encoded_layers=False")
        all_encoder_layers = []
        attacked_hidden_states = None
        calibrated_hidden_states = None
        all_attack_masks = []
        all_attention_prob = [] if return_attention_prob else None
        all_probs = [] if return_all_attention_prob else None
        for layer_idx, layer_module in enumerate(self.layer):
            rnd = _rnds[layer_idx] if _rnds is not None else None
            need_attacked = output_all_encoded_layers or layer_idx == len(self.layer) - 1
            outs = layer_module(hidden_states, attention_mask, return_attention_prob, return_all_attention_prob,
                                _rnd=rnd, _need_attacked=need_attacked,
                                _attack_upstream=layer_idx > 0 or not state_of(self).prune_dead_work,
                                _rows=_last_rows if layer_idx == len(self.layer) - 1 else None)
            attacked_hidden_states, calibrated_hidden_states, attack_mask, combined_attention_prob = outs[:4]
            hidden_states = calibrated_hidden_states
            all_attack_masks.append(attack_mask)
            if output_all_encoded_layers:
                all_encoder_layers.append((attacked_hidden_states, calibrated_hidden_states))
            if return_attention_prob:
                all_attention_prob.append(combined_attention_prob)
            if return_all_attention_prob:
                all_probs.append(outs[4])
        if not output_all_encoded_layers:
            all_encoder_layers.append((attacked_hidden_states, calibrated_hidden_states))
        if return_all_attention_prob:
            return all_encoder_layers, all_attack_masks, all_probs
        if return_attention_prob:
            return all_encoder_layers, all_attack_masks, all_attention_prob
        return all_encoder_layers, all_attack_masks
```

### ac_tsr_amd/linear.py

```python
from __future__ import annotations

import torch
import torch.nn.functional as F

from .state import DEFAULT as _DEFAULT_STATE, state_of


def _sum_rows(x, dim):
    from .ops import sum_rows
    return sum_rows(x, dim)



def _split(m: int) -> int:
    best = 1
    for s in range(2, 129):
        if m % s == 0 and m // s >= 128:
            best = s
    return best


class _SkinnyLinear(torch.autograd.Function):
    @staticmethod
    def forward(ctx, x, weight, bias, is_attack, state):
# ... 24 lines not shown
    if not x.is_cuda or not torch.is_grad_enabled():
        return layer(x)
    return _SkinnyLinear.apply(x, layer.weight, layer.bias, getattr(layer, "_acattn_attack", False), state_of(layer))


class _Projections(torch.autograd.Function):

    @staticmethod
    def forward(ctx, x, wq, bq, wk, bk, wv, bv, waq, baq, wak, bak, wg, bg, attack_upstream, state):
        mq, mk, mv = F.linear(x, wq, bq), F.linear(x, wk, bk), F.linear(x, wv, bv)
        qa, ka = F.linear(mq, waq, baq), F.linear(mk, wak, bak)
        gate = F.linear(mq, wg, bg) if wg is not None else None
        ctx.save_for_backward(x, mq, mk, wq, wk, wv, waq, wak, wg if wg is not None else x.new_empty(0))
        ctx.has_gate = wg is not None
        ctx.attack_upstream = attack_upstream
        ctx.state = state
        ctx.set_materialize_grads(False)
        return mq, mk, mv, qa, ka, gate

    @staticmethod
    def backward(ctx, dmq, dmk, dmv, dqa, dka, dgate):
        from .ops import linear_wgrad
        x, mq, mk, wq, wk, wv, waq, wak, wg = ctx.saved_tensors
        H = x.shape[-1]
        two = lambda t: None if t is None else t.reshape(-1, t.shape[-1])
        x2, mq2, mk2 = two(x), two(mq), two(mk)
        dmq, dmk, dmv, dqa, dka, dgate = (two(t) for t in (dmq, dmk, dmv, dqa, dka, dgate))

        def acc_(total, g, w):
            if g is None:
                return total
            return g @ w if total is None else total.addmm_(g, w)

        grads = [None] * 12
        others = not ctx.state.attack_pass_only
        attack = not ctx.state.calibrated_pass_only
        need_dx = ctx.needs_input_grad[0] and (others or ctx.attack_upstream)
        dx = dmq_t = dmk_t = None
        if need_dx or others:
            dmq_t = acc_(acc_(dmq, dqa, waq), dgate if ctx.has_gate else None, wg)
            dmk_t = acc_(dmk, dka, wak)
        if need_dx:
            dx = acc_(acc_(acc_(None, dmq_t, wq), dmk_t, wk), dmv, wv)
            dx = dx.view_as(x) if dx is not None else None
        jobs = []

        def params(slot, inp, g, want):
            if want and g is not None and (ctx.needs_input_grad[slot] or ctx.needs_input_grad[slot + 1]):
                jobs.append((slot, inp, g, ctx.needs_input_grad[slot + 1]))

        params(1, x2, dmq_t, others)
        params(3, x2, dmk_t, others)
        params(5, x2, dmv, others)
        params(7, mq2, dqa, attack)
        params(9, mk2, dka, attack)
        if ctx.has_gate:
            params(11, mq2, dgate, others)
        if jobs:
            from .ops import linear_wgrad_grouped
            for (slot, _, _, _), (gw, gb) in zip(jobs, linear_wgrad_grouped([(i, g, wb) for _, i, g, wb in jobs], ctx.state)):
                grads[slot - 1], grads[slot] = gw, gb
        return (dx, *grads, None, None)


FUSED_PROJECTIONS = True
PRODUCER_EXTRAS = True


class _FusedProjections(torch.autograd.Function):

    @staticmethod
    def _problem(x, wq, bq, wk, bk, wv, bv, waq, baq, wak, bak, wg, bg):
        from . import _lib
        from .ops import _ptr
        p = _lib.ProjProblem()
        p.rows, p.H, p.G = x.numel() // x.shape[-1], x.shape[-1], (wg.shape[0] if wg is not None else 0)
        p.x = _ptr(x)
        for name, t in (("wq", wq), ("bq", bq), ("wk", wk), ("bk", bk), ("wv", wv), ("bv", bv), ("waq", waq), ("baq", baq),
                        ("wak", wak), ("bak", bak), ("wg", wg), ("bg", bg)):
            setattr(p, name, _ptr(t))
        return p

    @staticmethod
    def forward(ctx, x, wq, bq, wk, bk, wv, bv, waq, baq, wak, bak, wg, bg, attack_upstream, state, spatial=None):
        import ctypes as C
        from . import _lib
        from .ops import _ptr, _stream
        x = x.contiguous()
        params = [None if t is None else t.contiguous() for t in (wq, bq, wk, bk, wv, bv, waq, baq, wak, bak, wg, bg)]
        p = _FusedProjections._problem(x, *params)
        mq, mk, mv, qa, ka = (torch.empty_like(x) for _ in range(5))
        gate = x.new_empty(*x.shape[:-1], p.G) if wg is not None else None
        out = _lib.ProjOut()
        out.mq, out.mk, out.mv, out.qa, out.ka, out.gate = (_ptr(t) for t in (mq, mk, mv, qa, ka, gate))
        affine = None
        keep = []
        if spatial is not None and x.dim() == 3:
            w_order, b_order, w_dist, b_dist, n_heads = spatial
            B, L, H = x.shape
            affine = _affine_workspace(state, x.device, B, n_heads, L)
            keep = [t.detach().reshape(-1).contiguous() for t in (w_order, b_order, w_dist, b_dist)]
            p.w_order, p.b_order, p.w_dist, p.b_dist = (_ptr(t) for t in keep)
            p.n_heads, p.L = n_heads, L
            out.affine = _ptr(affine)
            out.gate_prob = 1 if gate is not None else 0
        _lib.check(_lib.load().acattn_projections_fwd(C.byref(p), C.byref(out), _stream()), "projections_fwd")
        ctx.save_for_backward(x, mq, mk, *(t if t is not None else x.new_empty(0) for t in params))
        ctx.has_gate = wg is not None
        ctx.attack_upstream = attack_upstream
        ctx.state = state
        ctx.set_materialize_grads(False)
        if affine is not None:
            ctx.mark_non_differentiable(affine)
        return mq, mk, mv, qa, ka, gate, x.view_as(x), affine

    @staticmethod
    def backward(ctx, dmq, dmk, dmv, dqa, dka, dgate, d_res=None, _d_affine=None):
        import ctypes as C
        from . import _lib
        from .ops import _ptr, _stream, linear_wgrad_grouped
        x, mq, mk = ctx.saved_tensors[:3]
        params = [t if t.numel() else None for t in ctx.saved_tensors[3:]]
        two = lambda t: None if t is None else t.reshape(-1, t.shape[-1])
        con = lambda t: None if t is None else t.contiguous()
        dmq, dmk, dmv, dqa, dka, dgate, d_res = (con(t) for t in (dmq, dmk, dmv, dqa, dka, dgate, d_res))
        if not ctx.has_gate:
            dgate = None
        others = not ctx.state.attack_pass_only
        attack = not ctx.state.calibrated_pass_only
        need_dx = ctx.needs_input_grad[0] and (others or ctx.attack_upstream)
        dx = dmq_t = dmk_t = None
        if all(t is None for t in (dmq, dmk, dmv, dqa, dka, dgate)):
            dx = d_res if need_dx else None
        elif need_dx or others:
            io = _lib.ProjBwdIO()
            io.dmq, io.dmk, io.dmv, io.dqa, io.dka, io.dgate = (_ptr(t) for t in (dmq, dmk, dmv, dqa, dka, dgate))
            io.dx_init = _ptr(d_res) if need_dx else None
            dmq_t = dmq if dmq is not None else torch.empty_like(x)
            dmk_t = dmk if dmk is not None else torch.empty_like(x)
            dx = torch.empty_like(x) if need_dx else None
            io.dmq_total, io.dmk_total, io.dx = _ptr(dmq_t), _ptr(dmk_t), _ptr(dx)
            p = _FusedProjections._problem(x, *params)
            ws_bytes = int(_lib.load().acattn_projections_bwd_workspace_bytes(C.byref(p)))
            ws = torch.empty(ws_bytes // 4, device=x.device, dtype=torch.float32) if ws_bytes > 0 else None
            io.workspace = _ptr(ws)
            _lib.check(_lib.load().acattn_projections_bwd(C.byref(p), C.byref(io), _stream()), "projections_bwd")
        grads = [None] * 12
        jobs = []

        def want(slot, inp, g, on):
            if on and g is not None and (ctx.needs_input_grad[slot] or ctx.needs_input_grad[slot + 1]):
                jobs.append((slot, two(inp), two(g), ctx.needs_input_grad[slot + 1]))

        want(1, x, dmq_t, others)
        want(3, x, dmk_t, others)
        want(5, x, dmv, others)
        want(7, mq, dqa, attack)
        want(9, mk, dka, attack)
        if ctx.has_gate:
            want(11, mq, dgate, others)
        if jobs:
            for (slot, _, _, _), (gw, gb) in zip(jobs, linear_wgrad_grouped([(i, g, wb) for _, i, g, wb in jobs], ctx.state)):
                grads[slot - 1], grads[slot] = gw, gb
        return (dx, *grads, None, None, None)


def _affine_workspace(state, device, B, n_heads, L):
    if getattr(state, "_frozen", True):
        return torch.zeros(B, n_heads, 4, 16 * ((L + 15) // 16), device=device, dtype=torch.float32)
    key = (str(device), B, n_heads, L)
    ws = state.affine_ws.get(key)
    if ws is None:
        ws = state.affine_ws[key] = torch.zeros(B, n_heads, 4, 16 * ((L + 15) // 16), device=device, dtype=torch.float32)
    return ws


def projections(x, query, key, value, attack_query, attack_key, gate=None, attack_upstream=True, spatial=None):
    node = _Projections if torch.is_grad_enabled() else None
    if x.is_cuda and FUSED_PROJECTIONS and x.dtype == torch.float32 and all(
            m.bias is not None for m in (query, key, value, attack_query, attack_key) + ((gate,) if gate is not None else ())):
        from . import _lib
        if _lib.load().acattn_projections_supported(x.shape[-1], gate.out_features if gate is not None else 0):
            node = _FusedProjections
    if not x.is_cuda or node is None:
        mq, mk, mv = query(x), key(x), value(x)
        return mq, mk, mv, attack_query(mq), attack_key(mk), (gate(mq) if gate is not None else None), x, {}
    args = (x, query.weight, query.bias, key.weight, key.bias, value.weight, value.bias,
            attack_query.weight, attack_query.bias, attack_key.weight, attack_key.bias,
            gate.weight if gate is not None else None, gate.bias if gate is not None else None,
            attack_upstream, state_of(query))
    if node is _FusedProjections:
        if not PRODUCER_EXTRAS or (spatial is not None and any(t is None for t in spatial[:4])):
            spatial = None
        *out, affine = node.apply(*args, spatial)
        extras = {} if affine is None else {"affine": affine, "gate_is_prob": gate is not None}
        return (*out, extras)
    out = node.apply(*args)
    return (*out, x, {})


class _FusedQKV(torch.autograd.Function):

    @staticmethod
    def forward(ctx, x, wq, bq, wk, bk, wv, bv, state, spatial=None):
        import ctypes as C
        from . import _lib
        from .ops import _ptr, _stream
        x = x.contiguous()
        params = [t.contiguous() for t in (wq, bq, wk, bk, wv, bv)]
        p = _lib.ProjProblem()
        p.rows, p.H, p.G, p.x = x.numel() // x.shape[-1], x.shape[-1], 0, _ptr(x)
        p.wq, p.bq, p.wk, p.bk, p.wv, p.bv = (_ptr(t) for t in params)
        mq, mk, mv = (torch.empty_like(x) for _ in range(3))
        out = _lib.ProjOut()
        out.mq, out.mk, out.mv = _ptr(mq), _ptr(mk), _ptr(mv)
        affine = None
        keep = []
        if spatial is not None and x.dim() == 3:
            w_order, b_order, w_dist, b_dist, n_heads = spatial
            B, L, H = x.shape
            affine = _affine_workspace(state, x.device, B, n_heads, L)
            keep = [t.detach().reshape(-1).contiguous() for t in (w_order, b_order, w_dist, b_dist)]
            p.w_order, p.b_order, p.w_dist, p.b_dist = (_ptr(t) for t in keep)
            p.n_heads, p.L = n_heads, L
            out.affine = _ptr(affine)
        _lib.check(_lib.load().acattn_projections_qkv_fwd(C.byref(p), C.byref(out), _stream()), "projections_qkv_fwd")
        ctx.save_for_backward(x, *params)
        ctx.state = state
        ctx.set_materialize_grads(False)
        if affine is not None:
            ctx.mark_non_differentiable(affine)
        return mq, mk, mv, x.view_as(x), affine

    @staticmethod
    def backward(ctx, dmq, dmk, dmv, d_res=None, _d_affine=None):
        import ctypes as C
        from . import _lib
        from .ops import _ptr, _stream, linear_wgrad_grouped
        x, wq, bq, wk, bk, wv, bv = ctx.saved_tensors
        two = lambda t: None if t is None else t.reshape(-1, t.shape[-1])
        con = lambda t: None if t is None else t.contiguous()
        dmq, dmk, dmv, d_res = (con(t) for t in (dmq, dmk, dmv, d_res))
        if ctx.state.attack_pass_only:
            return (None,) * 9
        dx = None
        if ctx.needs_input_grad[0]:
            if all(t is None for t in (dmq, dmk, dmv)):
                dx = d_res
            else:
                p = _lib.ProjProblem()
                p.rows, p.H, p.G, p.x = x.numel() // x.shape[-1], x.shape[-1], 0, _ptr(x)
                p.wq, p.bq, p.wk, p.bk, p.wv, p.bv = (_ptr(t) for t in (wq, bq, wk, bk, wv, bv))
                p.waq, p.baq, p.wak, p.bak = p.wq, p.bq, p.wk, p.bk
                io = _lib.ProjBwdIO()
                io.dmq, io.dmk, io.dmv, io.dx_init = _ptr(dmq), _ptr(dmk), _ptr(dmv), _ptr(d_res)
                dx = torch.empty_like(x)
                io.dx = _ptr(dx)
                _lib.check(_lib.load().acattn_projections_bwd(C.byref(p), C.byref(io), _stream()), "projections_bwd (qkv)")
        grads = [None] * 6
        jobs = [(slot, two(x), two(g), ctx.needs_input_grad[slot + 1]) for slot, g in ((1, dmq), (3, dmk), (5, dmv))
                if g is not None and (ctx.needs_input_grad[slot] or ctx.needs_input_grad[slot + 1])]
        if jobs:
            for (slot, _, _, _), (gw, gb) in zip(jobs, linear_wgrad_grouped([(i, g, wb) for _, i, g, wb in jobs], ctx.state)):
                grads[slot - 1], grads[slot] = gw, gb
        return (dx, *grads, None, None)


def projections_qkv(x, query, key, value, spatial=None):
    if x.is_cuda and FUSED_PROJECTIONS and x.dtype == torch.float32 and all(m.bias is not None for m in (query, key, value)):
        from . import _lib
        if _lib.load().acattn_projections_qkv_supported(x.shape[-1]):
            if not PRODUCER_EXTRAS or (spatial is not None and any(t is None for t in spatial[:4])):
                spatial = None
            mq, mk, mv, x_res, affine = _FusedQKV.apply(x, query.weight, query.bias, key.weight, key.bias, value.weight,
                                                         value.bias, state_of(query), spatial)
            return mq, mk, mv, x_res, ({} if affine is None else {"affine": affine})
    return skinny_linear(x, query), skinny_linear(x, key), skinny_linear(x, value), x, {}
# ... 66 lines not shown
```

### ac_tsr_amd/tail.py

```python
from __future__ import annotations

import ctypes as C

import torch
import torch.nn.functional as F

from . import _lib, fused_ln, ops
from .ops import _ptr, _stream
from .state import state_of

FUSED_KERNEL = True
FUSED_MAX_HIDDEN = 128


def _tail_problem(c, x, wd, bd, g1, b1, w1, bb1, w2, bb2, g2, b2, eps1, eps2, p1, p2, k1, k2, seed1, seed2, seed_t,
                  rows=None):
    p = _lib.TailProblem()
    H, I = wd.shape[0], w1.shape[0]
    p.rows, p.H, p.I = c.numel() // H, H, I
    if rows is not None:
        p.rows, p.src_index, p.src_R, p.src_L = rows.numel(), _ptr(rows), rows.shape[-1], c.shape[-2]
    p.ctx, p.x = _ptr(c), _ptr(x)
    p.wd, p.bd, p.g1, p.b1 = _ptr(wd), _ptr(bd), _ptr(g1), _ptr(b1)
    p.w1, p.bb1, p.w2, p.bb2, p.g2, p.b2 = _ptr(w1), _ptr(bb1), _ptr(w2), _ptr(bb2), _ptr(g2), _ptr(b2)
    p.eps1, p.eps2, p.p1, p.p2 = float(eps1), float(eps2), float(p1), float(p2)
    p.keep1, p.keep2 = _ptr(k1), _ptr(k2)
    p.seed1, p.seed2 = seed1 & 0xFFFFFFFFFFFFFFFF, seed2 & 0xFFFFFFFFFFFFFFFF
    p.seed_device = _ptr(seed_t)
    return p


class _FusedLayerTail(torch.autograd.Function):
    @staticmethod
    def forward(ctx, c, x, wd, bd, g1, b1, w1, bb1, w2, bb2, g2, b2, eps1, eps2, p1, p2, keep1, keep2, seed1, seed2,
                seed_tensor, state, pick=None):
        ctx.state = state
        c, x = c.contiguous(), x.contiguous()
        params = tuple(t.contiguous() for t in (wd, bd, g1, b1, w1, bb1, w2, bb2, g2, b2))
        k1 = None if keep1 is None else keep1.to(torch.uint8).contiguous()
        k2 = None if keep2 is None else keep2.to(torch.uint8).contiguous()
        H, I = c.shape[-1], w1.shape[0]
        if pick is not None:
            pick = pick.contiguous()
            assert c.dim() == 3 and x.shape == c.shape and pick.dtype == torch.int64 and pick.shape[0] == c.shape[0]
            out_shape = (*pick.shape, H)
        else:
            out_shape = c.shape
        rows = 1
        for d in out_shape[:-1]:
            rows *= d
        new = lambda *shape: torch.empty(*shape, device=c.device, dtype=torch.float32)
        h1, a, h3, out = (new(*out_shape) for _ in range(4))
        st1, st2, act = new(rows, 2), new(rows, 2), new(rows, I)
        dgelu = new(rows, I) if (H > 64 and any(ctx.needs_input_grad)) else None
        p = _tail_problem(c, x, *params, eps1, eps2, p1, p2, k1, k2, seed1, seed2, seed_tensor, pick)
        lib = _lib.load()
        planes = None
        nbytes = int(lib.acattn_layer_tail_split_bytes(H, I, rows))
        if nbytes > 0:
            planes = new(nbytes // 4)
            _lib.check(lib.acattn_layer_tail_split_weights(C.byref(p), _ptr(planes), _stream()), "layer_tail_split_weights")
            p.split_planes = _ptr(planes)
        sv = _lib.TailSaved()
        sv.h1, sv.st1, sv.a, sv.act, sv.h3, sv.st2, sv.out = (_ptr(t) for t in (h1, st1, a, act, h3, st2, out))
        sv.gelu_grad = _ptr(dgelu)
        _lib.check(lib.acattn_layer_tail_fwd(C.byref(p), C.byref(sv), _stream()), "layer_tail_fwd")
        empty = c.new_empty(0)
        ctx.save_for_backward(c, x, h1, st1, a, act, h3, st2, *params, k1 if k1 is not None else empty,
                              k2 if k2 is not None else empty, seed_tensor if seed_tensor is not None else empty,
                              pick if pick is not None else empty, dgelu if dgelu is not None else empty,
                              planes if planes is not None else empty)
        ctx.args = (eps1, eps2, p1, p2, k1 is not None, k2 is not None, seed1, seed2, seed_tensor is not None,
                    pick is not None)
        return out

    @staticmethod
    def backward(ctx, d_out):
        c, x, h1, st1, a, act, h3, st2 = ctx.saved_tensors[:8]
        params = ctx.saved_tensors[8:18]
        k1, k2, seed_t, pick, dgelu, planes = ctx.saved_tensors[18:]
        eps1, eps2, p1, p2, has_k1, has_k2, seed1, seed2, has_seed_t, has_pick = ctx.args
        k1, k2, seed_t = (k1 if has_k1 else None), (k2 if has_k2 else None), (seed_t if has_seed_t else None)
        pick = pick if has_pick else None
        want_params = not ctx.state.attack_pass_only
        need_c, need_x = ctx.needs_input_grad[0], ctx.needs_input_grad[1]
        lib = _lib.load()
        rows, H, I = act.shape[0], c.shape[-1], act.shape[-1]
        new = lambda *shape: torch.empty(*shape, device=c.device, dtype=torch.float32)
        d_out = d_out.contiguous()
        p = _tail_problem(c, x, *params, eps1, eps2, p1, p2, k1, k2, seed1, seed2, seed_t, pick)
        p.split_planes = _ptr(planes) if planes.numel() else None
        sv = _lib.TailSaved()
        sv.h1, sv.st1, sv.a, sv.act, sv.h3, sv.st2 = (_ptr(t) for t in (h1, st1, a, act, h3, st2))
        sv.gelu_grad = _ptr(dgelu) if dgelu.numel() else None
        io = _lib.TailBwdIO()
        if pick is not None and need_c and need_x:
            d_c, d_x = torch.zeros(2, *c.shape, device=c.device, dtype=c.dtype).unbind(0)
        else:
            alloc = torch.zeros_like if pick is not None else torch.empty_like
            d_c = alloc(c) if need_c else None
            d_x = alloc(x) if need_x else None
        io.d_out, io.d_ctx, io.d_x = _ptr(d_out), _ptr(d_c), _ptr(d_x)
        d_h1 = d_h2 = d_h3 = part = None
        if want_params:
            d_h1, d_h2, d_h3 = new(rows, H), new(rows, I), new(rows, H)
            part = new(int(lib.acattn_layer_tail_bwd_partial_rows_for(rows, H)), 4 * H)
            io.d_h1, io.d_h2, io.d_h3, io.dgb_part = _ptr(d_h1), _ptr(d_h2), _ptr(d_h3), _ptr(part)
        ws_bytes = int(lib.acattn_layer_tail_bwd_workspace_bytes(H, I))
        ws = new(ws_bytes // 4) if ws_bytes > 0 else None
        io.workspace = _ptr(ws)
        _lib.check(lib.acattn_layer_tail_bwd(C.byref(p), C.byref(sv), C.byref(io), _stream()), "layer_tail_bwd")
        grads = [None] * 10
        if want_params:
            two = lambda t: t.reshape(-1, t.shape[-1])
            c_rows = two(c) if pick is None else c.gather(1, pick.unsqueeze(-1).expand(-1, -1, H)).view(-1, H)
            (gwd, gbd), (gw1, gb1), (gw2, gb2) = ops.linear_wgrad_grouped(
                [(c_rows, d_h1, True), (two(a), d_h2, True), (act, d_h3, True)], ctx.state)
            gb = ops.sum_rows0(part, ctx.state).view(4, H)
            grads = [gwd, gbd, gb[0], gb[1], gw1, gb1, gw2, gb2, gb[2], gb[3]]
            ctx.state.watch(gb, grads[2], grads[3], grads[8], grads[9])
        return (d_c, d_x, *grads, None, None, None, None, None, None, None, None, None, None, None)



class _LayerTail(torch.autograd.Function):
    @staticmethod
    def forward(ctx, c, x, wd, bd, g1, b1, w1, bb1, w2, bb2, g2, b2, eps1, eps2, p1, p2, keep1, keep2, seed1, seed2,
                seed_tensor, state):
        ctx.state = state
        c, x = c.contiguous(), x.contiguous()
        k1 = None if keep1 is None else keep1.to(torch.uint8).contiguous()
        k2 = None if keep2 is None else keep2.to(torch.uint8).contiguous()
        h1 = F.linear(c, wd, bd)
        a, st1 = fused_ln.forward_raw(h1, x, g1, b1, eps1, p1, k1, seed1, seed_tensor)
        h2 = F.linear(a, w1, bb1)
        act = F.gelu(h2)
        h3 = F.linear(act, w2, bb2)
        out, st2 = fused_ln.forward_raw(h3, a, g2, b2, eps2, p2, k2, seed2, seed_tensor)
        empty = c.new_empty(0)
        ctx.save_for_backward(c, x, h1, st1, a, h2, act, h3, st2, wd, g1, b1, w1, w2, g2, b2,
                              k1 if k1 is not None else empty, k2 if k2 is not None else empty,
                              seed_tensor if seed_tensor is not None else empty)
        ctx.args = (eps1, eps2, p1, p2, k1 is not None, k2 is not None, seed1, seed2, seed_tensor is not None)
        return out

    @staticmethod
    def backward(ctx, d_out):
        (c, x, h1, st1, a, h2, act, h3, st2, wd, g1, b1, w1, w2, g2, b2, k1, k2, seed_t) = ctx.saved_tensors
        eps1, eps2, p1, p2, has_k1, has_k2, seed1, seed2, has_seed_t = ctx.args
        k1, k2, seed_t = (k1 if has_k1 else None), (k2 if has_k2 else None), (seed_t if has_seed_t else None)
        params = not ctx.state.attack_pass_only
        two = lambda t: t.reshape(-1, t.shape[-1])
        d_h3, d_a, part2 = fused_ln.backward_raw(h3, a, g2, b2, eps2, p2, k2, seed2, seed_t, st2, d_out, want_gb=params)
        d_act = two(d_h3) @ w2
        d_h2 = torch.ops.aten.gelu_backward(d_act.view_as(h2), h2)
        two(d_a).addmm_(two(d_h2), w1)
        need_c, need_x = ctx.needs_input_grad[0], ctx.needs_input_grad[1]
        d_h1, d_x, part1 = fused_ln.backward_raw(h1, x, g1, b1, eps1, p1, k1, seed1, seed_t, st1, d_a, want_dres=need_x,
                                                 want_gb=params)
        d_c = (two(d_h1) @ wd).view_as(c) if need_c else None
        grads = [None] * 10
        if params:
            (gwd, gbd), (gw1, gb1), (gw2, gb2) = ops.linear_wgrad_grouped(
                [(two(c), two(d_h1), True), (two(a), two(d_h2), True), (two(act), two(d_h3), True)], ctx.state)
            gb = ops.sum_rows(torch.stack((part1, part2)), 1)
            grads = [gwd, gbd, gb[0, 0], gb[0, 1], gw1, gb1, gw2, gb2, gb[1, 0], gb[1, 1]]
        return (d_c, d_x, *grads, None, None, None, None, None, None, None, None, None, None)


def supported(att, ffn) -> bool:
    return (ffn.intermediate_act_fn == ffn.gelu and fused_ln.supported(att.dense.out_features)
            and att.dense.bias is not None and ffn.dense_1.bias is not None and ffn.dense_2.bias is not None)


def fused_supported(att, ffn) -> bool:
    H = att.dense.out_features
    if H > FUSED_MAX_HIDDEN:
        return False
    return FUSED_KERNEL and bool(_lib.load().acattn_layer_tail_supported(H, ffn.dense_1.out_features))


def layer_tail(ctx_layer, input_tensor, att, ffn, keep_out=None, keep_ffn=None, pick=None):
    training = att.training
    p1 = att.out_dropout.p if (training or keep_out is not None) else 0.0
    p2 = ffn.dropout.p if (training or keep_ffn is not None) else 0.0
    state = state_of(att)
    seed1 = state.draw_seed() if (p1 > 0 and keep_out is None) else 0
    seed2 = state.draw_seed() if (p2 > 0 and keep_ffn is None) else 0
    seed_t = state.seed_tensor if (keep_out is None and keep_ffn is None) else None
    extra = ()
    node = _LayerTail
    if fused_supported(att, ffn):
        node, extra = _FusedLayerTail, (pick,)
    else:
        assert pick is None, "row selection inside the tail needs the fused node"
    return node.apply(ctx_layer, input_tensor, att.dense.weight, att.dense.bias, att.LayerNorm.weight,
                            att.LayerNorm.bias, ffn.dense_1.weight, ffn.dense_1.bias, ffn.dense_2.weight,
                            ffn.dense_2.bias, ffn.LayerNorm.weight, ffn.LayerNorm.bias, att.LayerNorm.eps,
                            ffn.LayerNorm.eps, p1, p2, keep_out, keep_ffn, seed1, seed2, seed_t, state, *extra)
```

### include/acattn.h

```cpp
#ifndef ACATTN_H_
#define ACATTN_H_

#include <stdint.h>

#ifdef __cplusplus
extern "C" {
#endif

#define ACATTN_ABI_VERSION 32

enum {
  ACATTN_MASK_STRUCTURED = 0,
  ACATTN_MASK_DENSE_LL = 1,
  ACATTN_MASK_DENSE_L = 2
};

enum { ACATTN_COMBINE_FIXED = 0, ACATTN_COMBINE_GATE = 1, ACATTN_COMBINE_ANNEALING = 2 };

enum { ACATTN_RICH_NONE = 0, ACATTN_RICH_FIXED = 1, ACATTN_RICH_TRAINABLE = 2 };

enum {
  ACATTN_RNG_EXPLICIT = 0,
  ACATTN_RNG_COUNTER = 1
};

#define ACATTN_NSTAT 8

typedef struct acattn_problem {
  int32_t B, L, H, n_heads;
  const float* q;
  const float* k;
  const float* v;
  const float* qa;
  const float* ka;
  const float* gate_logits;
  int32_t mask_mode;
  int32_t causal;
  const uint8_t* key_valid;
  const float* mask;
  const float* w_order;
  const float* b_order;
  const float* w_dist;
  const float* b_dist;
  const float* scalar;
  int32_t adversarial;
  int32_t combine_option;
  float anneal_rate;
  int32_t two_level;
  int32_t rich_combine;
  const float* rich_ratio;
  int32_t rng_mode;
  float p_drop;
  const float* noise;
  const uint8_t* keep_after;
  const uint8_t* keep_before;
  const uint8_t* keep_mask;
  uint64_t seed;
  const uint64_t* seed_device;
  const float* affine;
  int32_t gate_is_prob;
} acattn_problem;

typedef struct acattn_fwd_out {
  float* ctx_attacked;
  float* ctx_calibrated;
  float* attack_mask;
  float* row_stats;
  float* after_spatial;
  float* before_spatial;
  float* perturbed_attention;
  float* calibrated_attention;
  float* penalty_part;
} acattn_fwd_out;

typedef struct acattn_bwd_io {
  const float* attack_mask;
  const float* row_stats;
  const float* d_ctx_attacked;
  const float* d_ctx_calibrated;
  const float* d_attack_mask;
  float* dq;
  float* dk;
  float* dv;
  float* dqa;
  float* dka;
  float* dgate_logits;
  float* dw_order_part;
  float* dw_dist_part;
  float* dsmall_part;
  int32_t part_stride;
  const uint32_t* active_qblocks;
  int32_t attack_only;
// ... 106 lines not shown
                                  int32_t n_masks, const float* direction, float* d_out, int32_t n_dir, void* stream);
#define ACATTN_MAX_MASKS 8
int acattn_mask_penalty_partial_multi(const float* const* m, int32_t n_masks, int64_t n, float* part, void* stream);
int acattn_mask_penalty_bwd_scaled_multi(const float* const* m, const float* norms, const float* d_loss, float scale, int64_t n,
                                         float* const* d_m, int32_t n_masks, void* stream);

int64_t acattn_linear_wgrad_workspace_bytes(int64_t M, int32_t K, int32_t N);
int acattn_linear_wgrad(const float* x, const float* dy, int64_t M, int32_t K, int32_t N, void* workspace, float* dw,
                        float* db, void* stream);

#define ACATTN_WGRAD_MAX_GROUP 8
int acattn_linear_wgrad_grouped(const float* const* x, const float* const* dy, const int32_t* K, const int32_t* N,
                                float* const* dw, float* const* db, int32_t n_items, int64_t M, void* workspace,
                                void* stream);

#define ACATTN_WGRAD_MAX_REDUCE 32
#define ACATTN_SUMROWS_MAX_DEFER 8
int acattn_linear_wgrad_grouped_partial(const float* const* x, const float* const* dy, const int32_t* K, const int32_t* N,
                                        const int32_t* want_bias, int32_t n_items, int64_t M, void* workspace, int32_t* n_partials,
                                        int64_t* w_offset, int64_t* b_offset, void* stream);
int acattn_linear_wgrad_reduce_many(const float* const* part_w, const float* const* part_b, const int32_t* K, const int32_t* N,
                                    const int32_t* n_partials, float* const* dw, float* const* db, int32_t n_items,
                                    const float* const* sum_x, float* const* sum_out, const int32_t* sum_R, const int32_t* sum_C,
                                    int32_t n_sums, void* stream);

typedef struct acattn_tail_problem {
  int32_t rows, H, I;
  const float* ctx;
  const float* x;
  const float* wd;
  const float* bd;
  const float* g1;
  const float* b1;
  const float* w1;
  const float* bb1;
  const float* w2;
  const float* bb2;
  const float* g2;
  const float* b2;
  float eps1, eps2;
  float p1, p2;
  const uint8_t* keep1;
  const uint8_t* keep2;
  uint64_t seed1, seed2;
  const uint64_t* seed_device;
  const int64_t* src_index;
  int32_t src_R, src_L;
  const void* split_planes;
} acattn_tail_problem;

typedef struct acattn_tail_saved {
  float* h1;
  float* st1;
  float* a;
  float* act;
  float* h3;
  float* st2;
  float* out;
  float* gelu_grad;
} acattn_tail_saved;

typedef struct acattn_tail_bwd_io {
  const float* d_out;
  float* d_ctx;
  float* d_x;
  float* d_h1;
  float* d_h2;
  float* d_h3;
  float* dgb_part;
  void* workspace;
} acattn_tail_bwd_io;

int acattn_layer_tail_supported(int32_t H, int32_t I);
int acattn_layer_tail_fwd(const acattn_tail_problem* p, const acattn_tail_saved* saved, void* stream);
int acattn_layer_tail_bwd(const acattn_tail_problem* p, const acattn_tail_saved* saved, const acattn_tail_bwd_io* io,
                          void* stream);
int32_t acattn_layer_tail_bwd_partial_rows(int32_t rows);
int32_t acattn_layer_tail_bwd_partial_rows_for(int32_t rows, int32_t H);
int64_t acattn_layer_tail_bwd_workspace_bytes(int32_t H, int32_t I);
int acattn_select_layer_tail_blocks(int nb);
int64_t acattn_layer_tail_split_bytes(int32_t H, int32_t I, int32_t rows);
int acattn_layer_tail_split_weights(const acattn_tail_problem* p, void* planes, void* stream);

typedef struct acattn_proj_problem {
  int32_t rows, H, G;
  const float* x;
  const float *wq, *bq;
  const float *wk, *bk;
  const float *wv, *bv;
  const float *waq, *baq;
  const float *wak, *bak;
  const float *wg, *bg;
  const float *w_order, *b_order, *w_dist, *b_dist;
  int32_t n_heads, L;
} acattn_proj_problem;

typedef struct acattn_proj_out {
  float *mq, *mk, *mv, *qa, *ka;
  float* gate;
  float* affine;
  int32_t gate_prob;
} acattn_proj_out;

typedef struct acattn_proj_bwd_io {
  const float *dmq, *dmk, *dmv, *dqa, *dka;
  const float* dgate;
  float *dmq_total, *dmk_total, *dx;
  const float* dx_init;
  void* workspace;
} acattn_proj_bwd_io;

int acattn_projections_supported(int32_t H, int32_t G);
int64_t acattn_projections_bwd_workspace_bytes(const acattn_proj_problem* p);
int acattn_projections_fwd(const acattn_proj_problem* p, const acattn_proj_out* out, void* stream);
int acattn_projections_bwd(const acattn_proj_problem* p, const acattn_proj_bwd_io* io, void* stream);
int acattn_projections_qkv_supported(int32_t H);
int acattn_projections_qkv_fwd(const acattn_proj_problem* p, const acattn_proj_out* out, void* stream);

#define ACATTN_LINEAR_PRODUCTS_FP32 0
#define ACATTN_LINEAR_PRODUCTS_DEFAULT 1
int acattn_linear_products(int mode);

#define ACATTN_ADAM_MAX_TENSORS 64
typedef struct acattn_adam_group {
  int32_t n_tensors;
  float* param[ACATTN_ADAM_MAX_TENSORS];
  const float* grad[ACATTN_ADAM_MAX_TENSORS];
  float* exp_avg[ACATTN_ADAM_MAX_TENSORS];
  float* exp_avg_sq[ACATTN_ADAM_MAX_TENSORS];
  float* step[ACATTN_ADAM_MAX_TENSORS];
  int64_t numel[ACATTN_ADAM_MAX_TENSORS];
} acattn_adam_group;
int acattn_adam_step(const acattn_adam_group* g, double lr, double beta1, double beta2, double eps, double weight_decay,
                     int32_t* done, void* stream);

int acattn_calibrated_attention_bwd_gate_summed(const acattn_problem* p, const acattn_bwd_io* io);
int acattn_calibrated_attention_bwd_pair_supported(const acattn_problem* p, const acattn_bwd_io* io);

int acattn_abi_version(void);

const char* acattn_last_error(void);

int64_t acattn_fwd_algorithmic_bytes(const acattn_problem* p);

int acattn_calibrated_attention_fwd(const acattn_problem* p, const acattn_fwd_out* out, void* stream);

int acattn_spatial_affines(const acattn_problem* p, float* affine, void* stream);

int acattn_calibrated_attention_bwd(const acattn_problem* p, const acattn_bwd_io* io, void* stream);

int64_t acattn_calibrated_attention_bwd_workspace_bytes(const acattn_problem* p);

typedef struct acattn_spatial_bwd_io {
  const float* d_ctx;
  float* dq;
  float* dk;
  float* dv;
  float* dw_order_part;
  float* dw_dist_part;
  float* dsmall_part;
  int32_t part_stride;
  int32_t n_read_rows;
  const int64_t* read_rows;
  void* workspace;
} acattn_spatial_bwd_io;
int acattn_spatial_attention_bwd(const acattn_problem* p, const acattn_spatial_bwd_io* io, void* stream);
int64_t acattn_spatial_attention_bwd_workspace_bytes(const acattn_problem* p);

int acattn_rng_materialize(int32_t B, int32_t n_heads, int32_t L, uint64_t seed, float p_drop, float* noise,
                           uint8_t* keep_after, uint8_t* keep_mask, uint8_t* keep_before, void* stream);

enum {
  ACATTN_FWD_AUTO = 0,
  ACATTN_FWD_STREAM = 1,
  ACATTN_FWD_STAGED = 2,
  ACATTN_FWD_GENERAL = 3
};
// ... 14 lines not shown
```

Baseline: 481,700 user-sequences/sec.

## Pre-split layer weights once per step into shared planes for projections and tail

Adds a batched split-weights launch that converts all layers' tail and projection weights into precision-split plane images once per step. The fused tail and projection kernels then read these shared planes instead of re-splitting weights per call or staging them in LDS. New register-ring projection kernels stream plane fragments directly from global memory. The cost is an extra buffer and more kernel variants, and a risk of stale planes if the weights change after they are made.

```diff
diff --git a/ac_tsr_amd/_lib.py b/ac_tsr_amd/_lib.py
--- a/ac_tsr_amd/_lib.py
+++ b/ac_tsr_amd/_lib.py
@@ -9,7 +9,7 @@
 LIB_PATH = os.environ.get("ACATTN_LIB") or os.path.join(CSRC, "libacattn.so")
 HEADER_PATH = os.path.join(os.path.dirname(_HERE), "include", "acattn.h")
 
-ABI_VERSION = 32
+ABI_VERSION = 33
 MAX_MASKS = 8
 NSTAT = 8
 MASK_STRUCTURED, MASK_DENSE_LL, MASK_DENSE_L = 0, 1, 2
@@ -81,7 +81,7 @@
     _fields_ = [("rows", C.c_int32), ("H", C.c_int32), ("G", C.c_int32), ("x", _f), ("wq", _f), ("bq", _f), ("wk", _f),
                 ("bk", _f), ("wv", _f), ("bv", _f), ("waq", _f), ("baq", _f), ("wak", _f), ("bak", _f), ("wg", _f),
                 ("bg", _f), ("w_order", _f), ("b_order", _f), ("w_dist", _f), ("b_dist", _f), ("n_heads", C.c_int32),
-                ("L", C.c_int32)]
+                ("L", C.c_int32), ("split_planes", _f)]
 
 
 class ProjOut(C.Structure):
@@ -109,6 +109,14 @@
                 ("eps1", C.c_float), ("eps2", C.c_float), ("p1", C.c_float), ("p2", C.c_float), ("keep1", _f),
                 ("keep2", _f), ("seed1", C.c_uint64), ("seed2", C.c_uint64), ("seed_device", _f), ("src_index", _f),
                 ("src_R", C.c_int32), ("src_L", C.c_int32), ("split_planes", _f)]
+
+
+SPLIT_MAX_LAYERS = 8
+
+
+class SplitLayer(C.Structure):
+    _fields_ = [("wd", _f), ("w1", _f), ("w2", _f), ("I", C.c_int32), ("tail_planes", _f), ("wq", _f), ("wk", _f),
+                ("wv", _f), ("waq", _f), ("wak", _f), ("wg", _f), ("G", C.c_int32), ("proj_planes", _f)]
 
 
 class TailSaved(C.Structure):
@@ -169,6 +177,8 @@
     "acattn_select_layer_tail_blocks": (C.c_int, [C.c_int]),
     "acattn_layer_tail_split_bytes": (C.c_int64, [C.c_int32, C.c_int32, C.c_int32]),
     "acattn_layer_tail_split_weights": (C.c_int, [C.POINTER(TailProblem), C.c_void_p, C.c_void_p]),
+    "acattn_split_weights_many": (C.c_int, [C.POINTER(SplitLayer), C.c_int32, C.c_void_p]),
+    "acattn_projections_split_bytes": (C.c_int64, [C.c_int32, C.c_int32]),
     "acattn_adam_step": (C.c_int, [C.POINTER(AdamGroup), C.c_double, C.c_double, C.c_double, C.c_double, C.c_double, _f,
                                    C.c_void_p]),
     "acattn_dense_ce_fwd": (C.c_int, [_f, C.c_int64, C.c_int64, _f, _f, _f, C.c_void_p]),
diff --git a/ac_tsr_amd/csrc/acattn_api.hip b/ac_tsr_amd/csrc/acattn_api.hip
--- a/ac_tsr_amd/csrc/acattn_api.hip
+++ b/ac_tsr_amd/csrc/acattn_api.hip
@@ -239,6 +239,7 @@
     return fail("projections: input and parameters must be non-NULL");
   if ((p->wg != nullptr) != (p->bg != nullptr) || (p->wg != nullptr) != (p->G > 0))
     return fail("projections: gate weight, bias and width go together");
+  if (((uintptr_t)p->split_planes & 15) != 0) return fail("projections: split_planes must be 16-byte aligned");
   return 0;
 }
 
@@ -322,6 +323,27 @@
   if (p->H != 64 || (p->I != 256 && p->I != 128)) return fail("layer tail split planes: hidden 64, inner 256 or 128 only");
   if (((uintptr_t)planes & 15) != 0) return fail("layer tail split planes: planes must be 16-byte aligned");
   const int rc = acattn_launch_tail_split(*p, planes, (hipStream_t)stream);
+  if (rc > 0) snprintf(g_err, sizeof(g_err), "HIP launch failed: %s", hipGetErrorString((hipError_t)rc));
+  return rc;
+}
+
+int64_t acattn_projections_split_bytes(int32_t H, int32_t G) { return acattn_proj_split_bytes(H, G); }
+
+int acattn_split_weights_many(const acattn_split_layer* layers, int32_t n_layers, void* stream) {
+  if (!layers || n_layers < 1 || n_layers > ACATTN_SPLIT_MAX_LAYERS) return fail("split planes: 1 .. ACATTN_SPLIT_MAX_LAYERS layers");
+  for (int k = 0; k < n_layers; ++k) {
+    const acattn_split_layer& l = layers[k];
+    if (l.tail_planes) {
+      if (!l.wd || !l.w1 || !l.w2) return fail("split planes: tail planes need wd, w1 and w2");
+      if (l.I != 256 && l.I != 128) return fail("split planes: tail planes are for hidden 64, inner 256 or 128");
+    }
+    if (l.proj_planes) {
+      if (!l.wq || !l.wk || !l.wv || !l.waq || !l.wak) return fail("split planes: projection planes need the five square weights");
+      if ((l.wg != nullptr) != (l.G > 0) || l.G < 0 || l.G > 64) return fail("split planes: gate weight and width go together, at most 64 outputs");
+    }
+    if ((((uintptr_t)l.tail_planes | (uintptr_t)l.proj_planes) & 15) != 0) return fail("split planes: planes must be 16-byte aligned");
+  }
+  const int rc = acattn_launch_split_many(layers, n_layers, (hipStream_t)stream);
   if (rc > 0) snprintf(g_err, sizeof(g_err), "HIP launch failed: %s", hipGetErrorString((hipError_t)rc));
   return rc;
 }
diff --git a/ac_tsr_amd/csrc/acattn_common.h b/ac_tsr_amd/csrc/acattn_common.h
--- a/ac_tsr_amd/csrc/acattn_common.h
+++ b/ac_tsr_amd/csrc/acattn_common.h
@@ -283,6 +283,7 @@
 bool acattn_proj_supported(int H, int G);
 int64_t acattn_proj_bwd_ws_bytes(const acattn_proj_problem& p);
 int acattn_launch_proj_fwd(const acattn_proj_problem& p, const acattn_proj_out& o, hipStream_t stream);
+int64_t acattn_proj_split_bytes(int H, int G);
 bool acattn_proj_qkv_supported(int H);
 int acattn_launch_proj_qkv_fwd(const acattn_proj_problem& p, const acattn_proj_out& o, hipStream_t stream);
 int acattn_launch_proj_bwd(const acattn_proj_problem& p, const acattn_proj_bwd_io& io, hipStream_t stream);
@@ -293,6 +294,7 @@
 int acattn_select_tail_nb(int nb);
 int64_t acattn_tail_split_bytes(int H, int I, int rows);
 int acattn_launch_tail_split(const acattn_tail_problem& p, void* planes, hipStream_t stream);
+int acattn_launch_split_many(const acattn_split_layer* layers, int n_layers, hipStream_t stream);
 int acattn_launch_tail_fwd(const acattn_tail_problem& p, const acattn_tail_saved& s, hipStream_t stream);
 int acattn_launch_tail_bwd(const acattn_tail_problem& p, const acattn_tail_saved& s, const acattn_tail_bwd_io& io,
                            hipStream_t stream);
diff --git a/ac_tsr_amd/csrc/acattn_proj.hip b/ac_tsr_amd/csrc/acattn_proj.hip
--- a/ac_tsr_amd/csrc/acattn_proj.hip
+++ b/ac_tsr_amd/csrc/acattn_proj.hip
@@ -857,8 +857,9 @@
 }
 
 constexpr int SPW = 4;
-constexpr int SPLIT_MAT = 4 * 2 * 3 * 64;
+constexpr int SPLIT_MAT = SPLIT_SQ64;
 constexpr int SPLIT_LDS = 6 * SPLIT_MAT * (int)sizeof(b8);
+static_assert(6 * SPLIT_MAT == PROJ_PLANES_DIR, "the planes image of one direction is the LDS image");
 
 __device__ __forceinline__ int kperm(int s, int g, int j) { return 32 * s + 16 * (j >> 2) + 4 * g + (j & 3); }
 
@@ -1132,6 +1133,238 @@
   }
 }
 
+struct PlaneWeights {
+  const b8* img;
+  int lane;
+  b8 ring[4][2][3];
+  __device__ __forceinline__ void fetch(int m, int nt) {
+    const b8* mat = img + (size_t)m * SPLIT_MAT + lane;
+#pragma unroll
+    for (int s = 0; s < 2; ++s)
+#pragma unroll
+      for (int q = 0; q < 3; ++q) ring[nt][s][q] = mat[((nt * 2 + s) * 3 + q) * 64];
+  }
+  __device__ __forceinline__ void begin(int m) {
+#pragma unroll
+    for (int nt = 0; nt < 4; ++nt) fetch(m, nt);
+  }
+  template <int NB>
+  __device__ __forceinline__ void product(int next, const b8 (&b)[NB][2][3], f4 (&acc)[NB][4]) {
+#pragma unroll
+    for (int nt = 0; nt < 4; ++nt) {
+      PIN_ORDER();
+#pragma unroll
+      for (int s = 0; s < 2; ++s)
+#pragma unroll
+        for (int nb = 0; nb < NB; ++nb) acc[nb][nt] = mfma_split(ring[nt][s], b[nb][s], acc[nb][nt]);
+      if (next >= 0) fetch(next, nt);
+      PIN_ORDER();
+    }
+  }
+};
+
+struct LdsImage {
+  const b8* img;
+  int lane, cur;
+  __device__ __forceinline__ void begin(int m) {
+    cur = m;
+    __syncthreads();
+  }
+  template <int NB>
+  __device__ __forceinline__ void product(int next, const b8 (&b)[NB][2][3], f4 (&acc)[NB][4]) {
+    split_product<NB>(img + cur * SPLIT_MAT, lane, b, acc);
+    cur = next;
+  }
+};
+
+template <int NB>
+__device__ __forceinline__ void split_fwd_chain(const acattn_proj_problem& P, const acattn_proj_out& O, const Rows<NB>& W,
+                                                PlaneWeights& ws, int c, int g) {
+  const bool gate = P.wg != nullptr;
+  f4 xb[NB][4], m[NB][4], acc[NB][4];
+  b8 xs[NB][2][3], ms[NB][2][3];
+  f4 bias[4];
+  load_rows<4, NB>(P.x, W, g, xb);
+  load_bias<4>(P.bq, g, bias);
+  ws.begin(0);
+  split_rows<NB>(xb, xs);
+  set_rows<4, NB>(bias, m);
+  ws.product<NB>(1, xs, m);
+  store_rows<4, NB>(O.mq, W, g, m);
+  if (O.affine) write_affine<4, NB>(m, W, P, O.affine, 0, P.b_order[0], P.b_dist[0], 0, c, g);
+  split_rows<NB>(m, ms);
+  load_bias<4>(P.baq, g, bias);
+  set_rows<4, NB>(bias, acc);
+  ws.product<NB>(gate ? 2 : 3, ms, acc);
+  store_rows<4, NB>(O.qa, W, g, acc);
+  if (gate) {
+    const int GT = (P.G + 15) >> 4;
+#pragma unroll
+    for (int nt = 0; nt < 4; ++nt) {
+      f4 b;
+#pragma unroll
+      for (int r = 0; r < 4; ++r) b[r] = P.bg[min(16 * nt + 4 * g + r, P.G - 1)];
+#pragma unroll
+      for (int nb = 0; nb < NB; ++nb) acc[nb][nt] = b;
+    }
+    ws.product<NB>(3, ms, acc);
+#pragma unroll
+    for (int nt = 0; nt < 4; ++nt) {
+      if (nt >= GT) break;
+#pragma unroll
+      for (int nb = 0; nb < NB; ++nb) {
+        f4 v = acc[nb][nt];
+        if (O.gate_prob) v = gate_value(v, 0);
+        const int j0 = 16 * nt + 4 * g;
+        float* dst = O.gate + (size_t)W.row[nb] * P.G + j0;
+        if (W.ok[nb] && j0 + 3 < P.G) {
+          *(f4u*)dst = v;
+        } else if (W.ok[nb]) {
+#pragma unroll
+          for (int r = 0; r < 4; ++r)
+            if (j0 + r < P.G) dst[r] = v[r];
+        }
+      }
+    }
+  }
+  load_bias<4>(P.bk, g, bias);
+  set_rows<4, NB>(bias, m);
+  ws.product<NB>(4, xs, m);
+  store_rows<4, NB>(O.mk, W, g, m);
+  if (O.affine) write_affine<4, NB>(m, W, P, O.affine, 64 / P.n_heads, 0.f, 0.f, 2, c, g);
+  split_rows<NB>(m, ms);
+  load_bias<4>(P.bak, g, bias);
+  set_rows<4, NB>(bias, acc);
+  ws.product<NB>(5, ms, acc);
+  store_rows<4, NB>(O.ka, W, g, acc);
+  load_bias<4>(P.bv, g, bias);
+  set_rows<4, NB>(bias, acc);
+  ws.product<NB>(-1, xs, acc);
+  store_rows<4, NB>(O.mv, W, g, acc);
+}
+
+template <int NB>
+__global__ void __launch_bounds__(64, 2) proj_planes_fwd_kernel(const acattn_proj_problem P, const acattn_proj_out O) {
+  const int lane = threadIdx.x, c = lane & 15, g = lane >> 4;
+  const Rows<NB> W = wave_rows<NB>(P.rows);
+  PlaneWeights ws;
+  ws.img = (const b8*)P.split_planes;
+  ws.lane = lane;
+  split_fwd_chain<NB>(P, O, W, ws, c, g);
+}
+
+template <int MODE>
+struct SplitBwdFlags {
+  bool h_dmq, h_dmk, h_dmv, h_dqa, h_dka, h_dx, h_qt, h_kt, gate;
+  __device__ __forceinline__ SplitBwdFlags(const acattn_proj_problem& P, const acattn_proj_bwd_io& IO)
+      : h_dmq(MODE == 1 || (MODE == 0 && IO.dmq)), h_dmk(MODE == 1 || (MODE == 0 && IO.dmk)),
+        h_dmv(MODE == 1 || (MODE == 0 && IO.dmv)), h_dqa(MODE != 0 || IO.dqa), h_dka(MODE != 0 || IO.dka),
+        h_dx(MODE != 0 || IO.dx), h_qt(MODE != 0 || IO.dmq_total), h_kt(MODE != 0 || IO.dmk_total),
+        gate(MODE != 2 && IO.dgate && P.wg) {}
+  __device__ __forceinline__ int next(int m) const {
+    const bool need[6] = {h_dqa, gate, h_dx, h_dka, h_dx, h_dx && h_dmv};
+    int n = -1;
+#pragma unroll
+    for (int j = 5; j >= 0; --j)
+      if (j > m && need[j]) n = j;
+    return n;
+  }
+};
+
+template <int NB, int MODE, class WS>
+__device__ __forceinline__ void split_bwd_chain(const acattn_proj_problem& P, const acattn_proj_bwd_io& IO, const Rows<NB>& W,
+                                                const SplitBwdFlags<MODE>& F, WS& ws, int g) {
+  const bool h_dmq = F.h_dmq, h_dmk = F.h_dmk, h_dmv = F.h_dmv, h_dqa = F.h_dqa, h_dka = F.h_dka, h_dx = F.h_dx;
+  const bool h_qt = F.h_qt, h_kt = F.h_kt, gate = F.gate;
+  auto zero = [&](f4 (&v)[NB][4]) {
+#pragma unroll
+    for (int nb = 0; nb < NB; ++nb)
+#pragma unroll
+      for (int t = 0; t < 4; ++t) v[nb][t] = f4{0.f, 0.f, 0.f, 0.f};
+  };
+  f4 in[NB][4], dq[NB][4], dk[NB][4], dx[NB][4];
+  b8 bs[NB][2][3];
+  if (IO.dx_init && h_dx) load_rows<4, NB>(IO.dx_init, W, g, dx); else zero(dx);
+  if (h_dmq) load_rows<4, NB>(IO.dmq, W, g, dq); else zero(dq);
+  if (h_dqa) load_rows<4, NB>(IO.dqa, W, g, in);
+  const int first = F.next(-1);
+  if (first >= 0) ws.begin(first);
+
+  if (h_dqa) {
+    split_rows<NB>(in, bs);
+    ws.template product<NB>(F.next(0), bs, dq);
+  }
+  if (gate) {
+#pragma unroll
+    for (int nb = 0; nb < NB; ++nb)
+#pragma unroll
+      for (int s = 0; s < 2; ++s) {
+        float x[8];
+#pragma unroll
+        for (int j = 0; j < 8; ++j) {
+          const int k = kperm(s, g, j);
+          const float t = IO.dgate[(size_t)W.row[nb] * P.G + min(k, P.G - 1)];
+          x[j] = k < P.G ? t : 0.f;
+        }
+        split8(x, bs[nb][s][0], bs[nb][s][1], bs[nb][s][2]);
+      }
+    ws.template product<NB>(F.next(1), bs, dq);
+  }
+  if (h_qt) store_rows<4, NB>(IO.dmq_total, W, g, dq);
+  if (h_dx) {
+    split_rows<NB>(dq, bs);
+    ws.template product<NB>(F.next(2), bs, dx);
+  }
+
+  if (h_dmk) load_rows<4, NB>(IO.dmk, W, g, dk); else zero(dk);
+  if (h_dka) {
+    load_rows<4, NB>(IO.dka, W, g, in);
+    split_rows<NB>(in, bs);
+    ws.template product<NB>(F.next(3), bs, dk);
+  }
+  if (h_kt) store_rows<4, NB>(IO.dmk_total, W, g, dk);
+  if (h_dx) {
+    split_rows<NB>(dk, bs);
+    ws.template product<NB>(F.next(4), bs, dx);
+    if (h_dmv) {
+      load_rows<4, NB>(IO.dmv, W, g, in);
+      split_rows<NB>(in, bs);
+      ws.template product<NB>(-1, bs, dx);
+    }
+    store_rows<4, NB>(IO.dx, W, g, dx);
+  }
+}
+
+template <int NB, int MODE>
+__global__ void __launch_bounds__(64, NB == 1 ? 2 : 1) proj_planes_bwd_kernel(const acattn_proj_problem P, const acattn_proj_bwd_io IO) {
+  const SplitBwdFlags<MODE> F(P, IO);
+  const int lane = threadIdx.x, g = lane >> 4;
+  const Rows<NB> W = wave_rows<NB>(P.rows);
+  PlaneWeights ws;
+  ws.img = (const b8*)P.split_planes + PROJ_PLANES_DIR;
+  ws.lane = lane;
+  split_bwd_chain<NB, MODE>(P, IO, W, F, ws, g);
+}
+
+template <int NB, int MODE>
+__global__ void __launch_bounds__(64 * SPW) proj_fill_bwd_kernel(const acattn_proj_problem P, const acattn_proj_bwd_io IO) {
+  extern __shared__ b8 wsp[];
+  const SplitBwdFlags<MODE> F(P, IO);
+  const int lane = threadIdx.x & 63, wave = threadIdx.x >> 6, g = lane >> 4;
+  const Rows<NB> W = split_rows_of<NB>(P.rows, wave);
+  const b8* src = (const b8*)P.split_planes + PROJ_PLANES_DIR;
+  const bool need[6] = {F.h_dqa, F.gate, F.h_dx, F.h_dka, F.h_dx, F.h_dx && F.h_dmv};
+#pragma unroll
+  for (int m = 0; m < 6; ++m)
+    if (need[m]) {
+#pragma unroll
+      for (int i = 0; i < SPLIT_MAT / (64 * SPW); ++i)
+        wsp[m * SPLIT_MAT + i * 64 * SPW + threadIdx.x] = src[m * SPLIT_MAT + i * 64 * SPW + threadIdx.x];
+    }
+  LdsImage ws{wsp, lane, 0};
+  split_bwd_chain<NB, MODE>(P, IO, W, F, ws, g);
+}
+
 int rows_per_wave(int rows) {
   static const int forced = getenv("ACATTN_PROJ_ROWS_PER_WAVE") ? atoi(getenv("ACATTN_PROJ_ROWS_PER_WAVE")) : 0;
   if (forced == 16 || forced == 32) return forced;
@@ -1221,6 +1454,10 @@
   return g_linear_products;
 }
 bool use_split(const acattn_proj_problem& p) { return p.H == 64 && (!p.wg || p.G <= 64) && linear_products() == 1; }
+int64_t proj_split_bytes(int H, int G) {
+  if (H != 64 || G < 0 || G > 64 || linear_products() != 1) return 0;
+  return (int64_t)2 * PROJ_PLANES_DIR * (int64_t)sizeof(b8);
+}
 
 template <class K>
 bool allow_split_lds(K kern) {
@@ -1244,7 +1481,45 @@
   hipLaunchKernelGGL((proj_split_bwd_kernel<NB, MODE>), dim3(wgs), dim3(64 * SPW), SPLIT_LDS, stream, p, io);
   return (int)hipGetLastError();
 }
-}
+
+int planes_rows_per_wave(int rows, bool bwd) {
+  static const int forced[2] = {getenv("ACATTN_PROJ_PLANES_ROWS_FWD") ? atoi(getenv("ACATTN_PROJ_PLANES_ROWS_FWD")) : 0,
+                                getenv("ACATTN_PROJ_PLANES_ROWS_BWD") ? atoi(getenv("ACATTN_PROJ_PLANES_ROWS_BWD")) : 0};
+  if (forced[bwd] == 16 || forced[bwd] == 32) return forced[bwd];
+  return rows >= 16384 ? 32 : 16;
+}
+
+template <int NB>
+int launch_planes_fwd(const acattn_proj_problem& p, const acattn_proj_out& o, hipStream_t stream) {
+  const int blocks = (p.rows + 16 * NB - 1) / (16 * NB);
+  hipLaunchKernelGGL((proj_planes_fwd_kernel<NB>), dim3(blocks), dim3(64), 0, stream, p, o);
+  return (int)hipGetLastError();
+}
+
+template <int NB, int MODE>
+int launch_planes_bwd(const acattn_proj_problem& p, const acattn_proj_bwd_io& io, hipStream_t stream) {
+  const int blocks = (p.rows + 16 * NB - 1) / (16 * NB);
+  hipLaunchKernelGGL((proj_planes_bwd_kernel<NB, MODE>), dim3(blocks), dim3(64), 0, stream, p, io);
+  return (int)hipGetLastError();
+}
+
+template <int NB, int MODE>
+int launch_fill_bwd(const acattn_proj_problem& p, const acattn_proj_bwd_io& io, hipStream_t stream) {
+  static const bool lds_ok = allow_split_lds(proj_fill_bwd_kernel<NB, MODE>);
+  if (!lds_ok) return (int)hipErrorInvalidValue;
+  const int wgs = (p.rows + 16 * NB * SPW - 1) / (16 * NB * SPW);
+  hipLaunchKernelGGL((proj_fill_bwd_kernel<NB, MODE>), dim3(wgs), dim3(64 * SPW), SPLIT_LDS, stream, p, io);
+  return (int)hipGetLastError();
+}
+
+int planes_bwd_form() {
+  static const char* e = getenv("ACATTN_PROJ_PLANES_BWD");
+  static const int form = !e ? 0 : !strcmp(e, "fill") ? 1 : !strcmp(e, "lds") ? 2 : 0;
+  return form;
+}
+}
+
+int64_t acattn_proj_split_bytes(int H, int G) { return proj_split_bytes(H, G); }
 
 int acattn_linear_products_choice(int mode) {
   const int old = linear_products();
@@ -1256,6 +1531,8 @@
   if (p.H == 128) return launch_wide_fwd<128>(p, o, stream);
   if (p.H == 256) return launch_wide_fwd<256>(p, o, stream);
   const int rpw = rows_per_wave(p.rows), blocks = (p.rows + rpw - 1) / rpw;
+  if (p.split_planes && use_split(p))
+    return planes_rows_per_wave(p.rows, false) == 32 ? launch_planes_fwd<2>(p, o, stream) : launch_planes_fwd<1>(p, o, stream);
   if (use_split(p)) return rpw == 32 ? launch_split_fwd<2>(p, o, stream) : launch_split_fwd<1>(p, o, stream);
   if (rpw == 32)
     hipLaunchKernelGGL((proj_fwd_kernel<64, 2>), dim3(blocks), dim3(64), 0, stream, p, o);
@@ -1294,6 +1571,26 @@
   const bool all_in = attack && io.dmq && io.dmk && io.dmv && (io.dgate || !p.wg);
   const bool attack_only = attack && !io.dmq && !io.dmk && !io.dmv && !io.dgate;
   const int mode = !outs ? 0 : all_in ? 1 : attack_only ? 2 : 0;
+  if (p.split_planes && use_split(p) && planes_bwd_form() == 1) {
+    if (rpw == 32) {
+      if (mode == 1) return launch_fill_bwd<2, 1>(p, io, stream);
+      if (mode == 2) return launch_fill_bwd<2, 2>(p, io, stream);
+      return launch_fill_bwd<2, 0>(p, io, stream);
+    }
+    if (mode == 1) return launch_fill_bwd<1, 1>(p, io, stream);
+    if (mode == 2) return launch_fill_bwd<1, 2>(p, io, stream);
+    return launch_fill_bwd<1, 0>(p, io, stream);
+  }
+  if (p.split_planes && use_split(p) && planes_bwd_form() == 0) {
+    if (planes_rows_per_wave(p.rows, true) == 32) {
+      if (mode == 1) return launch_planes_bwd<2, 1>(p, io, stream);
+      if (mode == 2) return launch_planes_bwd<2, 2>(p, io, stream);
+      return launch_planes_bwd<2, 0>(p, io, stream);
+    }
+    if (mode == 1) return launch_planes_bwd<1, 1>(p, io, stream);
+    if (mode == 2) return launch_planes_bwd<1, 2>(p, io, stream);
+    return launch_planes_bwd<1, 0>(p, io, stream);
+  }
   if (use_split(p)) {
     if (rpw == 32) {
       if (mode == 1) return launch_split_bwd<2, 1>(p, io, stream);
diff --git a/ac_tsr_amd/csrc/acattn_split.h b/ac_tsr_amd/csrc/acattn_split.h
--- a/ac_tsr_amd/csrc/acattn_split.h
+++ b/ac_tsr_amd/csrc/acattn_split.h
@@ -25,6 +25,9 @@
   }
 }
 
+constexpr int SPLIT_SQ64 = 4 * 2 * 3 * 64;
+constexpr int PROJ_PLANES_DIR = 6 * SPLIT_SQ64;
+
 __device__ __forceinline__ f4 mfma_split(const b8 (&a)[3], const b8 (&b)[3], f4 acc) {
 #define ACATTN_SPLIT_TERM(p, q) acc = mfma_bf(a[p], b[q], acc);
   ACATTN_SPLIT_TERMS(ACATTN_SPLIT_TERM)
diff --git a/ac_tsr_amd/csrc/acattn_tail.hip b/ac_tsr_amd/csrc/acattn_tail.hip
--- a/ac_tsr_amd/csrc/acattn_tail.hip
+++ b/ac_tsr_amd/csrc/acattn_tail.hip
@@ -518,6 +518,63 @@
   split8(x, p[0], p[1], p[2]);
 #pragma unroll
   for (int q = 0; q < 3; ++q) dst[((size_t)f * 3 + q) * 64 + lane] = p[q];
+}
+
+struct SplitManyArgs {
+  acattn_split_layer layer[ACATTN_SPLIT_MAX_LAYERS];
+};
+constexpr int SPLIT_MANY_PROJ_BLOCKS = 24, SPLIT_MANY_BLOCKS = SPLIT_MANY_PROJ_BLOCKS + 4 + 4 * (256 / 32);
+
+__device__ __forceinline__ void split_fragment(const float* w, b8* dst, int M, int K, int ld, int nv, bool T, int idx) {
+  const int KS = K / 32;
+  if (idx >= (M / 16) * KS * 64) return;
+  const int lane = idx & 63, f = idx >> 6, mt = f / KS, s = f % KS, c = lane & 15, g = lane >> 4, m = 16 * mt + c;
+  float x[8];
+#pragma unroll
+  for (int j = 0; j < 8; ++j) {
+    const int k = tail_kperm(s, g, j);
+    const int row = T ? k : m, col = T ? m : k;
+    const float t = w[(size_t)min(row, nv - 1) * ld + col];
+    x[j] = row < nv ? t : 0.f;
+  }
+  b8 p[3];
+  split8(x, p[0], p[1], p[2]);
+#pragma unroll
+  for (int q = 0; q < 3; ++q) dst[((size_t)f * 3 + q) * 64 + lane] = p[q];
+}
+
+__global__ void __launch_bounds__(256) split_many_kernel(const SplitManyArgs A) {
+  const acattn_split_layer& Ly = A.layer[blockIdx.y];
+  int b = blockIdx.x;
+  if (b < SPLIT_MANY_PROJ_BLOCKS) {
+    if (!Ly.proj_planes) return;
+    const int dir = b / 12, mi = (b % 12) >> 1, idx = (b & 1) * 256 + threadIdx.x;
+    const float* w = dir == 0 ? (mi == 0 ? Ly.wq : mi == 1 ? Ly.waq : mi == 2 ? Ly.wg : mi == 3 ? Ly.wk : mi == 4 ? Ly.wak : Ly.wv)
+                              : (mi == 0 ? Ly.waq : mi == 1 ? Ly.wg : mi == 2 ? Ly.wq : mi == 3 ? Ly.wak : mi == 4 ? Ly.wk : Ly.wv);
+    const bool is_gate = mi == (dir == 0 ? 2 : 1);
+    if (!w) return;
+    split_fragment(w, (b8*)Ly.proj_planes + (dir * 6 + mi) * SPLIT_SQ64, 64, 64, 64, is_gate ? Ly.G : 64, dir == 1, idx);
+    return;
+  }
+  if (!Ly.tail_planes) return;
+  b -= SPLIT_MANY_PROJ_BLOCKS;
+  const int I = Ly.I, RB = I / 32, SQ = SPLIT_SQ64, RECT = I * 64 * 3 / 8;
+  int mtx = 0;
+#pragma unroll
+  for (int k = 0; k < 6; ++k) {
+    const int nblk = k % 3 == 0 ? 2 : RB;
+    if (mtx == k && b >= nblk) {
+      b -= nblk;
+      ++mtx;
+    }
+  }
+  if (mtx >= 6) return;
+  const int which = mtx % 3;
+  const bool T = mtx >= 3;
+  const float* w = which == 0 ? Ly.wd : which == 1 ? Ly.w1 : Ly.w2;
+  const int M = which == 0 ? 64 : ((which == 1) != T ? I : 64), K = (which == 0 ? 64 * 64 : 64 * I) / M;
+  const int off = mtx == 0 ? 0 : mtx == 1 ? SQ : mtx == 2 ? SQ + RECT : mtx == 3 ? SQ + 2 * RECT : mtx == 4 ? 2 * SQ + 2 * RECT : 2 * SQ + 3 * RECT;
+  split_fragment(w, (b8*)Ly.tail_planes + off, M, K, T ? M : K, T ? K : M, T, b * 256 + threadIdx.x);
 }
 
 template <int KS>
@@ -1942,6 +1999,15 @@
   return -1;
 }
 
+int acattn_launch_split_many(const acattn_split_layer* layers, int n_layers, hipStream_t stream) {
+  static_assert(TailPlanes<256>::SQ == SPLIT_SQ64 && TailPlanes<128>::BWD_2 == 2 * SPLIT_SQ64 + 3 * (128 * 64 * 3 / 8), "");
+  SplitManyArgs args;
+  memset(&args, 0, sizeof(args));
+  for (int k = 0; k < n_layers; ++k) args.layer[k] = layers[k];
+  hipLaunchKernelGGL(split_many_kernel, dim3(SPLIT_MANY_BLOCKS, n_layers), dim3(256), 0, stream, args);
+  return (int)hipGetLastError();
+}
+
 int acattn_select_tail_nb(int nb) {
   const int prev = g_tail_nb;
   g_tail_nb = nb;
diff --git a/ac_tsr_amd/layers.py b/ac_tsr_amd/layers.py
--- a/ac_tsr_amd/layers.py
+++ b/ac_tsr_amd/layers.py
@@ -9,6 +9,7 @@
 import torch.nn.functional as F
 
 from . import fused_ln, ops
+from . import planes as planes_mod
 from . import tail
 from .linear import projections, projections_qkv, skinny_linear
 from .ops import AttentionConfig, ExplicitRandomness, StructuredMask
@@ -147,16 +148,17 @@
                                adversarial=self.adversarial, anneal_rate=rate)
 
     def forward(self, hidden_states, attention_mask, return_attention_prob=False, return_all_attention_prob=False,
-                _rnd=None, _need_attacked=True, _attack_upstream=True, _rows=None):
+                _rnd=None, _need_attacked=True, _attack_upstream=True, _rows=None, _planes=None):
         att = self.attack_attention
         cal = att.calibrator_params()
         if not self.adversarial:
             return self._forward_spatial_only(hidden_states, attention_mask, return_attention_prob, return_all_attention_prob,
-                                              _rnd, _rows)
+                                              _rnd, _rows, _planes)
         mq, mk, mv, qa, ka, gate_logits, hidden_res, extras = projections(
             hidden_states, att.query, att.key, att.value, att.attack_query_transform, att.attack_key_transform,
             self.gate if self.combine_option == 'gate' else None, attack_upstream=_attack_upstream,
-            spatial=(cal.get("w_order"), cal.get("b_order"), cal.get("w_dist"), cal.get("b_dist"), att.num_attention_heads))
+            spatial=(cal.get("w_order"), cal.get("b_order"), cal.get("w_dist"), cal.get("b_dist"), att.num_attention_heads),
+            planes=_planes)
         cfg = self._config()
         core_rnd = None
         if _rnd is not None:
@@ -185,10 +187,11 @@
             fused = one_launch or (ctx_layer.is_cuda and torch.is_grad_enabled() and tail.supported(att, self.feed_forward))
             if one_launch and _rows is not None:
                 return tail.layer_tail(ctx_layer, hidden_res, att, self.feed_forward, pick(keep_out), pick(keep_ffn),
-                                       pick=_rows)
+                                       pick=_rows, planes=_planes)
             ctx_layer, keep_out, keep_ffn = pick(ctx_layer), pick(keep_out), pick(keep_ffn)
             if fused:
-                return tail.layer_tail(ctx_layer, residual, att, self.feed_forward, keep_out, keep_ffn)
+                return tail.layer_tail(ctx_layer, residual, att, self.feed_forward, keep_out, keep_ffn,
+                                       planes=_planes if one_launch else None)
             return self.feed_forward(att.output(ctx_layer, residual, keep_out), keep_ffn)
 
         attacked_feedforward_output = None
@@ -210,7 +213,8 @@
                     all_attention_prob)
         return attacked_feedforward_output, calibrated_feedforward_output, attack_mask, combined_attention_prob
 
-    def _forward_spatial_only(self, hidden_states, attention_mask, return_attention_prob, return_all_attention_prob, _rnd, _rows):
+    def _forward_spatial_only(self, hidden_states, attention_mask, return_attention_prob, return_all_attention_prob, _rnd, _rows,
+                              _planes=None):
         if return_attention_prob or return_all_attention_prob:
             raise ValueError("adversarial=False: the spatial-only attention core has no probability dumps "
                              "(return_attention_prob / return_all_attention_prob need the adversarial calibrator)")
@@ -235,11 +239,13 @@
             index = _rows.unsqueeze(-1).expand(-1, -1, hidden_states.shape[-1])
             pick = lambda t: None if t is None else t.gather(1, index)
             if one_launch:
-                out = tail.layer_tail(ctx_cal, hidden_res, att, self.feed_forward, pick(keep_out), pick(keep_ffn), pick=_rows)
+                out = tail.layer_tail(ctx_cal, hidden_res, att, self.feed_forward, pick(keep_out), pick(keep_ffn), pick=_rows,
+                                      planes=_planes)
                 return None, out, None, None
             ctx_cal, hidden_res, keep_out, keep_ffn = pick(ctx_cal), pick(hidden_res), pick(keep_out), pick(keep_ffn)
         if one_launch or (can_tail and torch.is_grad_enabled()):
-            out = tail.layer_tail(ctx_cal, hidden_res, att, self.feed_forward, keep_out, keep_ffn)
+            out = tail.layer_tail(ctx_cal, hidden_res, att, self.feed_forward, keep_out, keep_ffn,
+                                  planes=_planes if one_launch else None)
         else:
             out = self.feed_forward(att.output(ctx_cal, hidden_res, keep_out), keep_ffn)
         return None, out, None, None
@@ -268,13 +274,15 @@
         all_attack_masks = []
         all_attention_prob = [] if return_attention_prob else None
         all_probs = [] if return_all_attention_prob else None
+        layer_planes = planes_mod.make(list(self.layer), hidden_states, _last_rows)
         for layer_idx, layer_module in enumerate(self.layer):
             rnd = _rnds[layer_idx] if _rnds is not None else None
             need_attacked = output_all_encoded_layers or layer_idx == len(self.layer) - 1
             outs = layer_module(hidden_states, attention_mask, return_attention_prob, return_all_attention_prob,
                                 _rnd=rnd, _need_attacked=need_attacked,
                                 _attack_upstream=layer_idx > 0 or not state_of(self).prune_dead_work,
-                                _rows=_last_rows if layer_idx == len(self.layer) - 1 else None)
+                                _rows=_last_rows if layer_idx == len(self.layer) - 1 else None,
+                                _planes=layer_planes[layer_idx])
             attacked_hidden_states, calibrated_hidden_states, attack_mask, combined_attention_prob = outs[:4]
             hidden_states = calibrated_hidden_states
             all_attack_masks.append(attack_mask)
diff --git a/ac_tsr_amd/linear.py b/ac_tsr_amd/linear.py
--- a/ac_tsr_amd/linear.py
+++ b/ac_tsr_amd/linear.py
@@ -130,7 +130,8 @@
         return p
 
     @staticmethod
-    def forward(ctx, x, wq, bq, wk, bk, wv, bv, waq, baq, wak, bak, wg, bg, attack_upstream, state, spatial=None):
+    def forward(ctx, x, wq, bq, wk, bk, wv, bv, waq, baq, wak, bak, wg, bg, attack_upstream, state, spatial=None,
+                planes=None):
         import ctypes as C
         from . import _lib
         from .ops import _ptr, _stream
@@ -152,6 +153,9 @@
             p.n_heads, p.L = n_heads, L
             out.affine = _ptr(affine)
             out.gate_prob = 1 if gate is not None else 0
+        ctx.planes = planes if (planes is not None and planes.proj is not None) else None
+        if ctx.planes is not None:
+            p.split_planes = _ptr(ctx.planes.proj)
         _lib.check(_lib.load().acattn_projections_fwd(C.byref(p), C.byref(out), _stream()), "projections_fwd")
         ctx.save_for_backward(x, mq, mk, *(t if t is not None else x.new_empty(0) for t in params))
         ctx.has_gate = wg is not None
@@ -189,6 +193,8 @@
             dx = torch.empty_like(x) if need_dx else None
             io.dmq_total, io.dmk_total, io.dx = _ptr(dmq_t), _ptr(dmk_t), _ptr(dx)
             p = _FusedProjections._problem(x, *params)
+            if ctx.planes is not None:
+                p.split_planes = _ptr(ctx.planes.proj)
             ws_bytes = int(_lib.load().acattn_projections_bwd_workspace_bytes(C.byref(p)))
             ws = torch.empty(ws_bytes // 4, device=x.device, dtype=torch.float32) if ws_bytes > 0 else None
             io.workspace = _ptr(ws)
@@ -210,7 +216,7 @@
         if jobs:
             for (slot, _, _, _), (gw, gb) in zip(jobs, linear_wgrad_grouped([(i, g, wb) for _, i, g, wb in jobs], ctx.state)):
                 grads[slot - 1], grads[slot] = gw, gb
-        return (dx, *grads, None, None, None)
+        return (dx, *grads, None, None, None, None)
 
 
 def _affine_workspace(state, device, B, n_heads, L):
@@ -223,7 +229,7 @@
     return ws
 
 
-def projections(x, query, key, value, attack_query, attack_key, gate=None, attack_upstream=True, spatial=None):
+def projections(x, query, key, value, attack_query, attack_key, gate=None, attack_upstream=True, spatial=None, planes=None):
     node = _Projections if torch.is_grad_enabled() else None
     if x.is_cuda and FUSED_PROJECTIONS and x.dtype == torch.float32 and all(
             m.bias is not None for m in (query, key, value, attack_query, attack_key) + ((gate,) if gate is not None else ())):
@@ -240,7 +246,7 @@
     if node is _FusedProjections:
         if not PRODUCER_EXTRAS or (spatial is not None and any(t is None for t in spatial[:4])):
             spatial = None
-        *out, affine = node.apply(*args, spatial)
+        *out, affine = node.apply(*args, spatial, planes)
         extras = {} if affine is None else {"affine": affine, "gate_is_prob": gate is not None}
         return (*out, extras)
     out = node.apply(*args)
diff --git a/ac_tsr_amd/planes.py b/ac_tsr_amd/planes.py
--- /dev/null
+++ b/ac_tsr_amd/planes.py
@@ -0,0 +1,80 @@
+from __future__ import annotations
+
+import ctypes as C
+import os
+
+import torch
+
+from . import _lib
+
+SHARED_PLANES = os.environ.get("ACATTN_SHARED_PLANES", "1") != "0"
+
+
+class LayerPlanes:
+    __slots__ = ("tail", "proj")
+
+    def __init__(self, tail=None, proj=None):
+        self.tail, self.proj = tail, proj
+
+
+def _plain(*tensors) -> bool:
+    return all(t.is_cuda and t.dtype == torch.float32 and t.is_contiguous() for t in tensors)
+
+
+def make(layers, hidden_states, last_rows=None):
+    n = len(layers)
+    if not SHARED_PLANES or n == 0 or not hidden_states.is_cuda or hidden_states.dtype != torch.float32:
+        return [None] * n
+    from . import linear, tail as tail_mod
+    from .ops import _ptr, _stream
+    lib = _lib.load()
+    H = hidden_states.shape[-1]
+    rows_all = hidden_states.numel() // H
+    jobs, sizes = [], []
+    for k, layer in enumerate(layers):
+        att, ffn = layer.attack_attention, layer.feed_forward
+        rows = last_rows.numel() if (last_rows is not None and k == n - 1) else rows_all
+        job = _lib.SplitLayer()
+        keep = []
+        t_bytes = p_bytes = 0
+        if (tail_mod.supported(att, ffn) and tail_mod.fused_supported(att, ffn)
+                and _plain(att.dense.weight, ffn.dense_1.weight, ffn.dense_2.weight)):
+            t_bytes = int(lib.acattn_layer_tail_split_bytes(H, ffn.dense_1.out_features, rows))
+            if t_bytes > 0:
+                job.wd, job.w1, job.w2 = (_ptr(w) for w in (att.dense.weight, ffn.dense_1.weight, ffn.dense_2.weight))
+                job.I = ffn.dense_1.out_features
+        gate = layer.gate if layer.combine_option == 'gate' else None
+        mods = (att.query, att.key, att.value, att.attack_query_transform, att.attack_key_transform)
+        every = mods + ((gate,) if gate is not None else ())
+        if (layer.adversarial and linear.FUSED_PROJECTIONS and all(m.bias is not None for m in every)
+                and _plain(*(m.weight for m in every))
+                and lib.acattn_projections_supported(H, gate.out_features if gate is not None else 0)):
+            p_bytes = int(lib.acattn_projections_split_bytes(H, gate.out_features if gate is not None else 0))
+            if p_bytes > 0:
+                job.wq, job.wk, job.wv, job.waq, job.wak = (_ptr(m.weight) for m in mods)
+                if gate is not None:
+                    job.wg, job.G = _ptr(gate.weight), gate.out_features
+        jobs.append(job)
+        sizes.append((t_bytes, p_bytes))
+    total = sum(t + p for t, p in sizes)
+    if total == 0:
+        return [None] * n
+    buf = torch.empty(total // 4, device=hidden_states.device, dtype=torch.float32)
+    holders, off = [], 0
+    for job, (t_bytes, p_bytes) in zip(jobs, sizes):
+        h = LayerPlanes()
+        if t_bytes:
+            h.tail = buf[off // 4:(off + t_bytes) // 4]
+            job.tail_planes = _ptr(h.tail)
+            off += t_bytes
+        if p_bytes:
+            h.proj = buf[off // 4:(off + p_bytes) // 4]
+            job.proj_planes = _ptr(h.proj)
+            off += p_bytes
+        holders.append(h if (t_bytes or p_bytes) else None)
+    live = [j for j, s in zip(jobs, sizes) if s[0] or s[1]]
+    for a in range(0, len(live), _lib.SPLIT_MAX_LAYERS):
+        chunk = live[a:a + _lib.SPLIT_MAX_LAYERS]
+        arr = (_lib.SplitLayer * len(chunk))(*chunk)
+        _lib.check(lib.acattn_split_weights_many(arr, len(chunk), _stream()), "split_weights_many")
+    return holders
diff --git a/ac_tsr_amd/tail.py b/ac_tsr_amd/tail.py
--- a/ac_tsr_amd/tail.py
+++ b/ac_tsr_amd/tail.py
@@ -33,7 +33,7 @@
 class _FusedLayerTail(torch.autograd.Function):
     @staticmethod
     def forward(ctx, c, x, wd, bd, g1, b1, w1, bb1, w2, bb2, g2, b2, eps1, eps2, p1, p2, keep1, keep2, seed1, seed2,
-                seed_tensor, state, pick=None):
+                seed_tensor, state, pick=None, shared=None):
         ctx.state = state
         c, x = c.contiguous(), x.contiguous()
         params = tuple(t.contiguous() for t in (wd, bd, g1, b1, w1, bb1, w2, bb2, g2, b2))
@@ -57,7 +57,11 @@
         lib = _lib.load()
         planes = None
         nbytes = int(lib.acattn_layer_tail_split_bytes(H, I, rows))
-        if nbytes > 0:
+        ctx.shared = None
+        if nbytes > 0 and shared is not None and shared.tail is not None and shared.tail.numel() * 4 == nbytes:
+            ctx.shared = shared
+            p.split_planes = _ptr(shared.tail)
+        elif nbytes > 0:
             planes = new(nbytes // 4)
             _lib.check(lib.acattn_layer_tail_split_weights(C.byref(p), _ptr(planes), _stream()), "layer_tail_split_weights")
             p.split_planes = _ptr(planes)
@@ -90,6 +94,8 @@
         d_out = d_out.contiguous()
         p = _tail_problem(c, x, *params, eps1, eps2, p1, p2, k1, k2, seed1, seed2, seed_t, pick)
         p.split_planes = _ptr(planes) if planes.numel() else None
+        if ctx.shared is not None:
+            p.split_planes = _ptr(ctx.shared.tail)
         sv = _lib.TailSaved()
         sv.h1, sv.st1, sv.a, sv.act, sv.h3, sv.st2 = (_ptr(t) for t in (h1, st1, a, act, h3, st2))
         sv.gelu_grad = _ptr(dgelu) if dgelu.numel() else None
@@ -119,7 +125,7 @@
             gb = ops.sum_rows0(part, ctx.state).view(4, H)
             grads = [gwd, gbd, gb[0], gb[1], gw1, gb1, gw2, gb2, gb[2], gb[3]]
             ctx.state.watch(gb, grads[2], grads[3], grads[8], grads[9])
-        return (d_c, d_x, *grads, None, None, None, None, None, None, None, None, None, None, None)
+        return (d_c, d_x, *grads, None, None, None, None, None, None, None, None, None, None, None, None)
 
 
 
@@ -180,7 +186,7 @@
     return FUSED_KERNEL and bool(_lib.load().acattn_layer_tail_supported(H, ffn.dense_1.out_features))
 
 
-def layer_tail(ctx_layer, input_tensor, att, ffn, keep_out=None, keep_ffn=None, pick=None):
+def layer_tail(ctx_layer, input_tensor, att, ffn, keep_out=None, keep_ffn=None, pick=None, planes=None):
     training = att.training
     p1 = att.out_dropout.p if (training or keep_out is not None) else 0.0
     p2 = ffn.dropout.p if (training or keep_ffn is not None) else 0.0
@@ -191,7 +197,7 @@
     extra = ()
     node = _LayerTail
     if fused_supported(att, ffn):
-        node, extra = _FusedLayerTail, (pick,)
+        node, extra = _FusedLayerTail, (pick, planes)
     else:
         assert pick is None, "row selection inside the tail needs the fused node"
     return node.apply(ctx_layer, input_tensor, att.dense.weight, att.dense.bias, att.LayerNorm.weight,
diff --git a/include/acattn.h b/include/acattn.h
--- a/include/acattn.h
+++ b/include/acattn.h
@@ -7,7 +7,7 @@
 extern "C" {
 #endif
 
-#define ACATTN_ABI_VERSION 32
+#define ACATTN_ABI_VERSION 33
 
 enum {
   ACATTN_MASK_STRUCTURED = 0,
@@ -280,6 +280,18 @@
 int64_t acattn_layer_tail_split_bytes(int32_t H, int32_t I, int32_t rows);
 int acattn_layer_tail_split_weights(const acattn_tail_problem* p, void* planes, void* stream);
 
+#define ACATTN_SPLIT_MAX_LAYERS 8
+typedef struct acattn_split_layer {
+  const float *wd, *w1, *w2;
+  int32_t I;
+  void* tail_planes;
+  const float *wq, *wk, *wv, *waq, *wak, *wg;
+  int32_t G;
+  void* proj_planes;
+} acattn_split_layer;
+int acattn_split_weights_many(const acattn_split_layer* layers, int32_t n_layers, void* stream);
+int64_t acattn_projections_split_bytes(int32_t H, int32_t G);
+
 typedef struct acattn_proj_problem {
   int32_t rows, H, G;
   const float* x;
@@ -291,6 +303,7 @@
   const float *wg, *bg;
   const float *w_order, *b_order, *w_dist, *b_dist;
   int32_t n_heads, L;
+  const void* split_planes;
 } acattn_proj_problem;
 
 typedef struct acattn_proj_out {
```

Result: faster. 491,000 user-sequences/sec (median of 6 runs) (+1.9%).
